# RapidAI/RapidDoc

Hardware: AMD Instinct MI355X
Metric: pages/sec (layout+OCR det/rec) (higher is better)
Workload: dtype f32

## Files before the change

### rapiddoc_amd/csrc/api.cpp

```cpp
#include "../../include/rapiddoc_mi355.h"

#include <mutex>
#include <string>

#include "engine.h"

namespace rd {
class FormulaDecoder;
FormulaDecoder* formula_decoder_create(int device, const void* blob, size_t nbytes);
void formula_decoder_destroy(FormulaDecoder* d);
int formula_decoder_decode(FormulaDecoder* d, const float* enc, int B, int S, int max_new, long long* ids, hipStream_t s);
int formula_decoder_max_new(FormulaDecoder* d);
}

struct rd_handle {
    rd::Engine* eng = nullptr;
    rd::FormulaDecoder* dec = nullptr;
    int device = 0;
    std::string kind;
    std::string err;
    std::string prof;
};

static thread_local std::string g_create_err;
// ... 209 lines not shown
    p.pages = pages; p.H = H; p.W = W; p.page_stride = (size_t)H * W * 3;
    p.descs = reinterpret_cast<const rd::LineCropDesc*>(descs); p.n = n;
    p.scratch = scratch; p.max_crop_pixels = (long)max_crop_pixels;
    if (rd::launch_line_warp(p, (hipStream_t)stream) != 0) return 1;
    return hipGetLastError() == hipSuccess ? 0 : 1;
}
int rd_line_resize_norm_batch(int device_id, const rd_line_crop_desc* descs, int n, const uint8_t* scratch, int out_h, int out_w_padded,
                              int swap_rb, float* out, void* stream) {
    if (!descs || !scratch || !out || n < 0 || out_h <= 0 || out_w_padded <= 0) return 1;
    if (hipSetDevice(device_id) != hipSuccess) return 1;
    rd::LineCropParams p{};
    p.descs = reinterpret_cast<const rd::LineCropDesc*>(descs); p.n = n;
    p.scratch = const_cast<uint8_t*>(scratch);
    p.dst = out; p.OH = out_h; p.OWp = out_w_padded; p.swap_rb = swap_rb;
    if (rd::launch_line_resize_norm(p, (hipStream_t)stream) != 0) return 1;
    return hipGetLastError() == hipSuccess ? 0 : 1;
}

int rd_ctc_collapse(int device_id, const int32_t* idx, const float* prob, int B, int T, const uint8_t* ctab, int max_len, int n_classes,
                    uint8_t* out, int row_bytes, void* stream) {
    if (!idx || !prob || !ctab || !out || B < 0 || T <= 0 || max_len <= 0 || n_classes <= 0) return 1;
    if (hipSetDevice(device_id) != hipSuccess) return 1;
    if (rd::launch_ctc_collapse(idx, prob, B, T, nullptr, ctab, max_len, n_classes, out, row_bytes, nullptr, nullptr, (hipStream_t)stream) != 0) return 1;
    return hipGetLastError() == hipSuccess ? 0 : 1;
}

int rd_ctc_collapse_lines(int device_id, const int32_t* idx, const float* prob, int n_lines, const int32_t* seg, int max_tokens,
                          const uint8_t* ctab, int max_len, int n_classes, uint8_t* out, int row_bytes, uint16_t* kept_cols, float* kept_conf,
                          void* stream) {
    if (!idx || !prob || !seg || !ctab || !out || n_lines < 0 || max_tokens <= 0 || max_len <= 0 || n_classes <= 0) return 1;
    if (hipSetDevice(device_id) != hipSuccess) return 1;
    if (rd::launch_ctc_collapse(idx, prob, n_lines, max_tokens, seg, ctab, max_len, n_classes, out, row_bytes, kept_cols, kept_conf,
                                (hipStream_t)stream) != 0)
        return 1;
    return hipGetLastError() == hipSuccess ? 0 : 1;
}

int rd_msdeform_attn(int device_id, const float* value, const int32_t* shapes, const int32_t* level_start, const float* loc, const float* attn,
                     float* out, int B, int S, int H, int D, int Q, int L, int P, void* stream) {
    if (!value || !shapes || !level_start || !loc || !attn || !out || B < 0 || S <= 0 || H <= 0 || D <= 0 || Q < 0 || L <= 0 || P <= 0 || H * D > 1024)
        return 1;
    if (hipSetDevice(device_id) != hipSuccess) return 1;
    rd::launch_msdeform_attn(value, shapes, level_start, loc, attn, out, B, S, H, D, Q, L, P, (hipStream_t)stream);
    return hipGetLastError() == hipSuccess ? 0 : 1;
}

int rd_topk_rows(int device_id, const float* scores, int rows, int n, int k, float* out_vals, int32_t* out_idx, void* stream) {
    if (!scores || !out_vals || !out_idx || rows < 0 || n <= 0 || k <= 0 || k > 1024 || k > n) return 1;
    if (hipSetDevice(device_id) != hipSuccess) return 1;
    rd::launch_topk_rows(scores, rows, n, k, out_vals, out_idx, (hipStream_t)stream);
    return hipGetLastError() == hipSuccess ? 0 : 1;
}

size_t rd_encoder_layer_workspace(int M, int Dm, int F) {
    if (M <= 0 || Dm <= 0 || F <= 0) return 0;
    return ((size_t)M * Dm * 3  + (size_t)M * 3 * Dm  + (size_t)M * F) * sizeof(float);
}

int rd_encoder_layer(int device_id, const float* x, const float* pos, int B, int T, int Dm, int heads, int F, int act, const float* in_w,
                     const float* in_b, const float* out_w, const float* out_b, const float* ln1_g, const float* ln1_b, const float* w1,
                     const float* b1, const float* w2, const float* b2, const float* ln2_g, const float* ln2_b, float eps, float* out, void* ws,
                     size_t ws_bytes, void* stream) {
    const int M = B * T;
    if (!x || !in_w || !out_w || !w1 || !w2 || !ln1_g || !ln1_b || !ln2_g || !ln2_b || !out || !ws || B <= 0 || T <= 0 || heads <= 0 ||
        Dm % heads != 0 || Dm % 4 != 0 || F % 4 != 0 || ws_bytes < rd_encoder_layer_workspace(M, Dm, F))
        return 1;
    const int hd = Dm / heads;
    if (hd != 16 && hd != 32) return 1;
    if (hipSetDevice(device_id) != hipSuccess) return 1;
    hipStream_t s = (hipStream_t)stream;
    float* xp = (float*)ws;
    float* att = xp + (size_t)M * Dm;
    float* y1 = att + (size_t)M * Dm;
    float* qkv = y1 + (size_t)M * Dm;
    float* ff = qkv + (size_t)M * 3 * Dm;
    auto gemm = [&](const float* a, int K, const float* w, const float* b, int N, float* y, int yld, int a_act, const float* res) {
        rd::ConvParams p{};
        p.x = a; p.xld = K; p.N = 1; p.H = 1; p.W = M; p.Cin = K;
        p.w = w; p.bias = b; p.y = y; p.yld = yld; p.OH = 1; p.OW = M; p.Cout = N;
        p.KH = p.KW = p.SH = p.SW = 1;
        p.res = res; p.rld = N;
        p.act = a_act; p.out_mode = rd::OUT_NHWC;
        p.M = M; p.K = K; p.Ng = N;
        rd::launch_conv_igemm(p, s);
    };
    try {
        const float* qk_in = x;
        if (pos) {
            rd::launch_add(x, Dm, pos, Dm, xp, Dm, M, Dm, s);
            qk_in = xp;
        }
        gemm(qk_in, Dm, in_w, in_b, 2 * Dm, qkv, 3 * Dm, rd::ACT_NONE, nullptr);
        gemm(x, Dm, in_w + (size_t)2 * Dm * Dm, in_b ? in_b + 2 * Dm : nullptr, Dm, qkv + 2 * Dm, 3 * Dm, rd::ACT_NONE, nullptr);
        rd::launch_attention(qkv, att, B, T, heads, hd, 1.0f / std::sqrt((float)hd), s);
        gemm(att, Dm, out_w, out_b, Dm, xp, Dm, rd::ACT_NONE, x);
        rd::launch_layernorm(xp, Dm, y1, Dm, ln1_g, ln1_b, M, Dm, eps, s);
        gemm(y1, Dm, w1, b1, F, ff, F, act, nullptr);
        gemm(ff, F, w2, b2, Dm, xp, Dm, rd::ACT_NONE, y1);
        rd::launch_layernorm(xp, Dm, out, Dm, ln2_g, ln2_b, M, Dm, eps, s);
    } catch (...) {
        return 1;
    }
    return hipGetLastError() == hipSuccess ? 0 : 1;
}

size_t rd_db_boxes_workspace(int B, int H, int W, int max_runs, int max_candidates) {
    (void)W;
    if (B <= 0 || H <= 0 || max_runs <= 0 || max_candidates <= 0) return 0;
    return rd::db_boxes_workspace_bytes(B, H, max_runs, max_candidates);
}
int rd_db_boxes_device(int device_id, const float* prob, int B, int H, int W, const int32_t* src_hw_dev, float thresh, float box_thresh,
                       float unclip_ratio, int use_dilation, int max_candidates, int max_runs, void* ws, size_t ws_bytes, rd_text_box* out,
                       int max_out, int32_t* n_out, void* stream) {
    if (!prob || !src_hw_dev || !ws || !out || !n_out || B < 0 || H <= 0 || W <= 0) return 1;
    if (hipSetDevice(device_id) != hipSuccess) return 1;
    if (rd::launch_db_boxes(prob, B, H, W, src_hw_dev, thresh, box_thresh, unclip_ratio, use_dilation, max_candidates, max_runs, ws, ws_bytes,
                            out, max_out, n_out, (hipStream_t)stream) != 0)
        return 1;
    return hipGetLastError() == hipSuccess ? 0 : 1;
}

float rd_debug_time_mixer(int C, int M, int variant, int iters, float* x, float* y, float* w1, float* b1, float* w2, float* b2) {
    rd::MixerParams p{};
    p.x = x; p.xld = C; p.y = y; p.yld = C; p.M = M; p.HW = M; p.C = C; p.gate = nullptr;
    p.w1 = w1; p.b1 = b1; p.w2 = w2; p.b2 = b2;
    hipEvent_t e0, e1;
    (void)hipEventCreate(&e0); (void)hipEventCreate(&e1);
    void* hbuf[4] = {nullptr, nullptr, nullptr, nullptr};
    int ws_abl = 0;
    if (variant >= 1000) { ws_abl = (variant - 1000) & ~0xff; variant = 200 + ((variant - 1000) & 0xff); }
    if (variant >= 600) variant -= 300;
    if (variant >= 300 && variant < 400) {
        std::vector<float> hw1((size_t)2 * C * C), hw2((size_t)2 * C * C);
        (void)hipMemcpy(hw1.data(), w1, hw1.size() * 4, hipMemcpyDeviceToHost);
        (void)hipMemcpy(hw2.data(), w2, hw2.size() * 4, hipMemcpyDeviceToHost);
        std::vector<uint16_t> img;
        float inv[2];
        rd::prepare_mixer_weights_res(hw1.data(), hw2.data(), C, img, inv);
        p.ws_inv1 = inv[0]; p.ws_inv2 = inv[1];
        (void)hipMalloc(&hbuf[0], img.size() * 2);
        (void)hipMemcpy(hbuf[0], img.data(), img.size() * 2, hipMemcpyHostToDevice);
        p.w1h = (const uint16_t*)hbuf[0];
    } else if (variant >= 200) {
        const bool pf = variant >= 400 && variant < 600;
        if (pf) variant -= 200;
        p.ws_pf = pf;
        p.dbg = (variant - 200) | ws_abl;
        std::vector<float> hw1((size_t)2 * C * C), hw2((size_t)2 * C * C);
        (void)hipMemcpy(hw1.data(), w1, hw1.size() * 4, hipMemcpyDeviceToHost);
        (void)hipMemcpy(hw2.data(), w2, hw2.size() * 4, hipMemcpyDeviceToHost);
        std::vector<uint16_t> img;
        float inv[2];
        rd::prepare_mixer_weights_ws(hw1.data(), hw2.data(), C, img, inv);
        p.ws_inv1 = inv[0]; p.ws_inv2 = inv[1];
        (void)hipMalloc(&hbuf[0], img.size() * 2);
        (void)hipMemcpy(hbuf[0], img.data(), img.size() * 2, hipMemcpyHostToDevice);
        p.w1h = (const uint16_t*)hbuf[0];
    } else if (variant >= 100) {
        p.dbg = variant - 100;
        std::vector<float> hw1((size_t)2 * C * C), hw2((size_t)2 * C * C);
        (void)hipMemcpy(hw1.data(), w1, hw1.size() * 4, hipMemcpyDeviceToHost);
        (void)hipMemcpy(hw2.data(), w2, hw2.size() * 4, hipMemcpyDeviceToHost);
        std::vector<uint16_t> v[4];
        rd::prepare_mixer_weights_h3(hw1.data(), hw2.data(), C, v[0], v[1], v[2], v[3]);
        for (int i = 0; i < 4; ++i) {
            (void)hipMalloc(&hbuf[i], v[i].size() * 2);
            (void)hipMemcpy(hbuf[i], v[i].data(), v[i].size() * 2, hipMemcpyHostToDevice);
        }
        p.w1h = (const uint16_t*)hbuf[0]; p.w1l = (const uint16_t*)hbuf[1];
        p.w2h = (const uint16_t*)hbuf[2]; p.w2l = (const uint16_t*)hbuf[3];
    }
    auto go = [&] {
        if (variant >= 300 && !p.ws_pf) rd::launch_mixer_fused_res(p, nullptr);
        else if (variant >= 200) rd::launch_mixer_fused_ws(p, nullptr);
        else if (variant >= 100) rd::launch_mixer_fused_h3(p, nullptr);
        else rd::launch_mixer_debug(p, variant, nullptr);
    };
    go();
    (void)hipEventRecord(e0, nullptr);
    for (int i = 0; i < iters; ++i) go();
    (void)hipEventRecord(e1, nullptr);
    (void)hipEventSynchronize(e1);
    float ms = 0.f;
    (void)hipEventElapsedTime(&ms, e0, e1);
    (void)hipEventDestroy(e0); (void)hipEventDestroy(e1);
    for (void* b : hbuf) if (b) (void)hipFree(b);
    return ms / iters;
}
static bool debug_h1_image(const float* w_dev, int N, int K, void** img_dev, float* inv) {
    if (!rd::gemm_h1_shape_ok(K, N)) return false;
    std::vector<float> hw((size_t)N * K);
    if (hipMemcpy(hw.data(), w_dev, hw.size() * 4, hipMemcpyDeviceToHost) != hipSuccess) return false;
    std::vector<uint16_t> img;
    *inv = rd::prepare_gemm_h1_weights(hw.data(), N, K, img);
    if (hipMalloc(img_dev, img.size() * 2) != hipSuccess) return false;
    (void)hipMemcpy(*img_dev, img.data(), img.size() * 2, hipMemcpyHostToDevice);
    return true;
}
float rd_debug_time_gemm(int M, int K, int N, int act, int iters, float* x, float* w, float* b, float* y, void* wh, void* wl) {
    rd::ConvParams p{};
    p.wh = (const uint16_t*)wh; p.wl = (const uint16_t*)wl;
    p.x = x; p.xld = K; p.N = 1; p.H = 1; p.W = M; p.Cin = K; p.w = w; p.bias = b; p.y = y; p.yld = N;
    p.OH = 1; p.OW = M; p.Cout = N; p.KH = p.KW = p.SH = p.SW = 1; p.act = act; p.out_mode = rd::OUT_NHWC;
    p.M = M; p.K = K; p.Ng = N;
    void* img = nullptr;
    float inv = 0.f;
    if (wh && debug_h1_image(w, N, K, &img, &inv)) { p.w1 = (const uint16_t*)img; p.w1_inv = inv; }
    hipEvent_t e0, e1;
    (void)hipEventCreate(&e0); (void)hipEventCreate(&e1);
    auto go = [&] { if (wh) rd::launch_conv_igemm_h3(p, nullptr); else rd::launch_conv_igemm(p, nullptr); };
    go();
    (void)hipEventRecord(e0, nullptr);
    for (int i = 0; i < iters; ++i) go();
    (void)hipEventRecord(e1, nullptr);
    (void)hipEventSynchronize(e1);
    float ms = 0.f;
    (void)hipEventElapsedTime(&ms, e0, e1);
    (void)hipEventDestroy(e0); (void)hipEventDestroy(e1);
    if (img) (void)hipFree(img);
    return ms / iters;
}
float rd_debug_gemm_h1(int M, int K, int N, int act, int iters, float* x, int xld, float* w, float* b, float* res, int rld, float* y, int yld,
                       int* range_out) {
    rd::ConvParams p{};
    p.x = x; p.xld = xld; p.N = 1; p.H = 1; p.W = M; p.Cin = K; p.w = w; p.bias = b; p.y = y; p.yld = yld;
    p.OH = 1; p.OW = M; p.Cout = N; p.KH = p.KW = p.SH = p.SW = 1; p.act = act; p.out_mode = rd::OUT_NHWC;
    p.res = res; p.rld = rld;
    p.M = M; p.K = K; p.Ng = N;
    void* img = nullptr;
    float inv = 0.f;
    if (!debug_h1_image(w, N, K, &img, &inv)) return -1.f;
    p.w1 = (const uint16_t*)img; p.w1_inv = inv;
    unsigned* flag = nullptr;
    (void)hipHostMalloc((void**)&flag, sizeof(unsigned), hipHostMallocMapped);
    *flag = 0;
    p.range_flag = flag;
    float ms = -1.f;
    if (rd::gemm_h1_applies(p)) {
        hipEvent_t e0, e1;
        (void)hipEventCreate(&e0); (void)hipEventCreate(&e1);
        rd::launch_gemm_h1(p, nullptr);
        (void)hipEventRecord(e0, nullptr);
        for (int i = 0; i < iters; ++i) rd::launch_gemm_h1(p, nullptr);
        (void)hipEventRecord(e1, nullptr);
        (void)hipEventSynchronize(e1);
        (void)hipEventElapsedTime(&ms, e0, e1);
        (void)hipEventDestroy(e0); (void)hipEventDestroy(e1);
        ms = iters > 0 ? ms / iters : 0.f;
    }
    (void)hipDeviceSynchronize();
    if (range_out) *range_out = (int)*flag;
    (void)hipHostFree(flag);
    (void)hipFree(img);
    return ms;
}

float rd_debug_conv(int N, int H, int W, int Cin, int Cout, int KH, int KW, int S, int PT, int PL, int PB, int PR, int act, int iters,
                    float* x, float* w, void* wh, void* wl, float* bias, float* res, float* y, int* used_direct) {
    rd::ConvParams p{};
    p.x = x; p.xld = Cin; p.N = N; p.H = H; p.W = W; p.Cin = Cin; p.w = w; p.bias = bias; p.y = y; p.yld = Cout;
    p.wh = (const uint16_t*)wh; p.wl = (const uint16_t*)wl;
    p.OH = (H + PT + PB - KH) / S + 1; p.OW = (W + PL + PR - KW) / S + 1; p.Cout = Cout;
    p.KH = KH; p.KW = KW; p.SH = p.SW = S; p.PT = PT; p.PL = PL; p.act = act; p.out_mode = rd::OUT_NHWC;
    p.res = res; p.rld = Cout;
    p.M = N * p.OH * p.OW; p.K = KH * KW * Cin; p.Ng = Cout;
    void* img3 = nullptr;
    if (wh && !(used_direct && *used_direct) && rd::conv3x3_h1_shape_ok(KH, KW, Cin, Cout)) {
        std::vector<float> hw((size_t)Cout * p.K);
        if (hipMemcpy(hw.data(), w, hw.size() * 4, hipMemcpyDeviceToHost) == hipSuccess) {
            std::vector<uint16_t> img;
            const float inv = rd::prepare_conv3x3_h1_weights(hw.data(), Cout, Cin, img);
            if (hipMalloc(&img3, img.size() * 2) == hipSuccess) {
                (void)hipMemcpy(img3, img.data(), img.size() * 2, hipMemcpyHostToDevice);
                p.w3 = (const uint16_t*)img3;
                p.w3_inv = inv;
            }
        }
    }
    const bool c3 = wh && rd::conv3x3_h1_applies(p);
    const bool force = used_direct && *used_direct == 1 && wh && rd::conv_direct_h3_supported(p);
    const bool force_stream = used_direct && *used_direct == 2 && wh && rd::conv_stream_h3_supported(p);
    if (used_direct) *used_direct = c3 ? 3 : force_stream ? 2 : (force || (wh && !rd::conv_stream_h3_applies(p) && rd::conv_direct_h3_applies(p))) ? 1
                                    : (wh && rd::conv_stream_h3_applies(p)) ? 2 : 0;
    hipEvent_t e0, e1;
    (void)hipEventCreate(&e0); (void)hipEventCreate(&e1);
    auto go = [&] {
        if (force_stream) rd::launch_conv_stream_h3(p, nullptr);
        else if (force) rd::launch_conv_direct_h3(p, nullptr);
        else if (wh) rd::launch_conv_igemm_h3(p, nullptr);
        else rd::launch_conv_igemm(p, nullptr);
    };
    go();
    (void)hipEventRecord(e0, nullptr);
    for (int i = 0; i < iters; ++i) go();
    (void)hipEventRecord(e1, nullptr);
    (void)hipEventSynchronize(e1);
    float ms = 0.f;
    (void)hipEventElapsedTime(&ms, e0, e1);
    (void)hipEventDestroy(e0); (void)hipEventDestroy(e1);
    if (img3) (void)hipFree(img3);
    return iters > 0 ? ms / iters : 0.f;
}

float rd_debug_stem34(int N, int H, int W, int Cin, int xld, int N1, int N2, int yld, int act3, int act4, int iters, float* x, float* w3, float* b3,
                      float* w4, float* b4, float* y, unsigned* range_flag) {
    if (!rd::stem34_shape_ok(Cin, N1, N2)) return -1.f;
    std::vector<float> h3((size_t)N1 * 9 * Cin), h4((size_t)N2 * N1), hb3((size_t)((N1 + 31) / 32) * 32, 0.f);
    if (hipMemcpy(h3.data(), w3, h3.size() * 4, hipMemcpyDeviceToHost) != hipSuccess) return -1.f;
    if (hipMemcpy(h4.data(), w4, h4.size() * 4, hipMemcpyDeviceToHost) != hipSuccess) return -1.f;
    if (hipMemcpy(hb3.data(), b3, (size_t)N1 * 4, hipMemcpyDeviceToHost) != hipSuccess) return -1.f;
    std::vector<uint16_t> i3, i4;
    float inv[2];
    rd::prepare_stem34_weights(h3.data(), h4.data(), Cin, N1, N2, i3, i4, inv);
    void *d3 = nullptr, *d4 = nullptr, *db3 = nullptr;
    if (hipMalloc(&d3, i3.size() * 2) != hipSuccess || hipMalloc(&d4, i4.size() * 2) != hipSuccess || hipMalloc(&db3, hb3.size() * 4) != hipSuccess) return -1.f;
    (void)hipMemcpy(d3, i3.data(), i3.size() * 2, hipMemcpyHostToDevice);
    (void)hipMemcpy(d4, i4.data(), i4.size() * 2, hipMemcpyHostToDevice);
    (void)hipMemcpy(db3, hb3.data(), hb3.size() * 4, hipMemcpyHostToDevice);
    rd::Stem34Params p{};
    p.x = x; p.xld = xld; p.N = N; p.H = H; p.W = W; p.Cin = Cin; p.y = y; p.yld = yld;
    p.OH = (H - 1) / 2 + 1; p.OW = (W - 1) / 2 + 1; p.N1 = N1; p.N2 = N2;
    p.w3 = (const uint16_t*)d3; p.w3_inv = inv[0]; p.b3 = (const float*)db3;
    p.w4 = (const uint16_t*)d4; p.w4_inv = inv[1]; p.b4 = b4;
    p.act3 = act3; p.act4 = act4; p.range_flag = range_flag;
    hipEvent_t e0, e1;
    (void)hipEventCreate(&e0); (void)hipEventCreate(&e1);
    rd::launch_stem34(p, nullptr);
    (void)hipEventRecord(e0, nullptr);
    for (int i = 0; i < iters; ++i) rd::launch_stem34(p, nullptr);
    (void)hipEventRecord(e1, nullptr);
    (void)hipEventSynchronize(e1);
    float ms = 0.f;
    (void)hipEventElapsedTime(&ms, e0, e1);
    (void)hipEventDestroy(e0); (void)hipEventDestroy(e1);
    (void)hipFree(d3); (void)hipFree(d4); (void)hipFree(db3);
    return iters > 0 ? ms / iters : 0.f;
}

float rd_debug_dwconv(int N, int H, int W, int C, int K, int SH, int act, int iters, float* x, float* w, float* bias, float* res, float* y,
                      const int32_t* line_w, float* gap, int* gap_chunks) {
    rd::DwParams p{};
    p.x = x; p.xld = C; p.N = N; p.H = H; p.W = W; p.C = C; p.w = w; p.bias = bias; p.y = y; p.yld = C;
    p.KH = p.KW = K; p.SH = SH; p.SW = 1; p.PT = p.PL = K / 2;
    p.OH = (H + 2 * p.PT - K) / SH + 1; p.OW = W; p.act = act; p.res = res; p.rld = C;
    const int chunks = rd::dwconv_gap_chunks(p);
    if (gap_chunks) *gap_chunks = chunks;
    p.gap_partial = chunks > 0 ? gap : nullptr; p.gap_chunks = chunks;
    p.line_w = line_w; p.line_w_stride = 1;
    if (gap_chunks && rd::dwconv_kxk_lds_applies(p)) *gap_chunks = -1;
    hipEvent_t e0, e1;
    (void)hipEventCreate(&e0); (void)hipEventCreate(&e1);
    rd::launch_dwconv(p, nullptr);
    (void)hipEventRecord(e0, nullptr);
    for (int i = 0; i < iters; ++i) rd::launch_dwconv(p, nullptr);
    (void)hipEventRecord(e1, nullptr);
    (void)hipEventSynchronize(e1);
    float ms = 0.f;
    (void)hipEventElapsedTime(&ms, e0, e1);
    (void)hipEventDestroy(e0); (void)hipEventDestroy(e1);
    return iters > 0 ? ms / iters : 0.f;
}

float rd_debug_time_ctc(int M, int K, int Ccls, int iters, float* x, float* wp, void* wh, void* wl, float* part, int32_t* idx, float* prob,
                        int nsplit_override, int* nsplit_out) {
    rd::CtcParams p{};
    p.x = x; p.xld = K; p.w = wp; p.M = M; p.K = K; p.C = Ccls; p.part = part;
    p.nsplit = nsplit_override > 0 ? nsplit_override : rd::ctc_head_nsplit(M, Ccls, wh != nullptr);
    p.idx = idx; p.prob = prob;
    p.wh = (const uint16_t*)wh; p.wl = (const uint16_t*)wl;
    if (nsplit_out) *nsplit_out = p.nsplit;
    hipEvent_t e0, e1;
    (void)hipEventCreate(&e0); (void)hipEventCreate(&e1);
    rd::launch_ctc_head(p, nullptr);
    (void)hipEventRecord(e0, nullptr);
    for (int i = 0; i < iters; ++i) rd::launch_ctc_head(p, nullptr);
    (void)hipEventRecord(e1, nullptr);
    (void)hipEventSynchronize(e1);
    float ms = 0.f;
    (void)hipEventElapsedTime(&ms, e0, e1);
    (void)hipEventDestroy(e0); (void)hipEventDestroy(e1);
    return ms / iters;
}

int rd_set_precision(rd_handle* h, const char* mode) {
    return guarded(h, [&] {
        RD_CHECK(h->eng, "precision modes apply to the network engines");
        const std::string m = mode ? mode : "";
        RD_CHECK(m == "auto" || m == "fp32" || m == "h3", "precision must be auto, fp32 or h3");
        h->eng->set_precision(m == "h3" ? rd::Engine::PREC_H3 : m == "fp32" ? rd::Engine::PREC_FP32 : rd::Engine::PREC_AUTO);
    });
}
int rd_range_status(rd_handle* h, void* stream) {
    int out = 0;
    const int rc = guarded(h, [&] { if (h->eng) out = h->eng->take_range_flag((hipStream_t)stream); });
    return rc != 0 ? -1 : out;
}

int rd_plan_stats(rd_handle* h, uint64_t* plans_built, uint64_t* graph_captures, uint64_t* graph_replays) {
    if (!h || !h->eng) return 1;
    if (plans_built) *plans_built = h->eng->plans_built();
    if (graph_captures) *graph_captures = h->eng->graph_captures();
    if (graph_replays) *graph_replays = h->eng->graph_replays();
    return 0;
}

int rd_set_profiling(rd_handle* h, int on) {
    return guarded(h, [&] { if (h->eng) h->eng->set_profiling(on != 0); });
}
const char* rd_profile_json(rd_handle* h) {
    if (!h || !h->eng) return "[]";
    h->prof = h->eng->profile_json();
    return h->prof.c_str();
}

}
```

### rapiddoc_amd/csrc/engine.cpp

```cpp
#include "engine.h"

#include <algorithm>
#include <cmath>
#include <cstdio>
#include <cstdlib>
#include <cstring>
#include <sstream>

namespace rd {

namespace {
struct JsonCur {
    const char* p;
    const char* end;
    void ws() {
        while (p < end && (*p == ' ' || *p == '\n' || *p == '\t' || *p == '\r')) ++p;
    }
    bool eat(char c) {
        ws();
        if (p < end && *p == c) { ++p; return true; }
        return false;
    }
    void expect(char c) {
        if (!eat(c)) throw Error(std::string("safetensors header: expected '") + c + "'");
// ... 383 lines not shown
            pb_->add_u16(key + "#w3", img);
            pb_->add(key + "#w3s", std::vector<float>{inv});
        }
        if (kh == 1 && kw == 1 && gemm_h1_shape_ok(K, cout)) {
            std::vector<uint16_t> img;
            const float inv = prepare_gemm_h1_weights(wf.data(), cout, K, img);
            pb_->add_u16(key + "#w1", img);
            pb_->add(key + "#w1s", std::vector<float>{inv});
        }
    }
}

bool Builder::mixer_takes_dw(const std::string& prefix, int C) const {
    if (!planning() || !(h3_ || mixer_h3_) || !mixer_res_fuses_dw(C)) return false;
    const std::string hkey = prefix + ".mixer#h3";
    static const bool ws_off = std::getenv("RD_MIXER_WS") && std::string(std::getenv("RD_MIXER_WS")) == "0";
    const bool split = pb_->has(hkey + ".w1h");
    const bool ws = split && !ws_off && pb_->has(hkey + ".ws");
    return split && !ws && pb_->has(hkey + ".res");
}

TView Builder::mixer_fused(const std::string& prefix, const TView& x, const TView* gate, const std::string* dw_key) {
    const std::string w1 = prefix + ".channel_conv1.convolution.weight", bn1 = prefix + ".channel_conv1.normalization";
    const std::string w2 = prefix + ".channel_conv2.convolution.weight", bn2 = prefix + ".channel_conv2.normalization";
    const int C = x.c;
    RD_CHECK(mixer_fused_supported(C), "mixer_fused: unsupported width");
    RD_CHECK(weight_dim(w1, 0) == 2 * C && weight_dim(w1, 1) == C && weight_dim(w2, 0) == C && weight_dim(w2, 1) == 2 * C,
             "mixer_fused: weight shapes: " + prefix);
    TView y = alloc(x.n, x.h, x.w, C);
    const std::string hkey = prefix + ".mixer#h3";
    if (!planning()) {
        fold_conv(w1, "", bn1);
        fold_conv(w2, "", bn2);
        const float* f1 = pb_->host_ptr(w1 + "|" + bn1 + "#w");
        const float* f2 = pb_->host_ptr(w2 + "|" + bn2 + "#w");
        const bool fits = fits_fp16_range(std::vector<float>(f1, f1 + (size_t)2 * C * C)) && fits_fp16_range(std::vector<float>(f2, f2 + (size_t)2 * C * C));
        if (!pb_->has(hkey + ".w1h") && fits) {
            std::vector<uint16_t> v[4];
            prepare_mixer_weights_h3(f1, f2, C, v[0], v[1], v[2], v[3]);
            pb_->add_u16(hkey + ".w1h", v[0]); pb_->add_u16(hkey + ".w1l", v[1]);
            pb_->add_u16(hkey + ".w2h", v[2]); pb_->add_u16(hkey + ".w2l", v[3]);
        }
        if (!pb_->has(hkey + ".res") && fits && mixer_res_supported(C)) {
            std::vector<uint16_t> img;
            float inv[2];
            prepare_mixer_weights_res(f1, f2, C, img, inv);
            pb_->add_u16(hkey + ".res", img);
            pb_->add(hkey + ".resinv", std::vector<float>{inv[0], inv[1]});
        }
        if (!pb_->has(hkey + ".ws") && fits && mixer_ws_preferred(C)) {
            std::vector<uint16_t> img;
            float inv[2];
            prepare_mixer_weights_ws(f1, f2, C, img, inv);
            pb_->add_u16(hkey + ".ws", img);
            pb_->add(hkey + ".wsinv", std::vector<float>{inv[0], inv[1]});
        }
        return y;
    }
    const bool split = (h3_ || mixer_h3_) && pb_->has(hkey + ".w1h");
    static const bool ws_off = std::getenv("RD_MIXER_WS") && std::string(std::getenv("RD_MIXER_WS")) == "0";
    const bool ws = split && !ws_off && pb_->has(hkey + ".ws");
    const bool res_k = split && !ws && mixer_res_supported(C) && pb_->has(hkey + ".res");
    MixerParams p{};
    if (res_k) {
        p.w1h = reinterpret_cast<const uint16_t*>(pb_->ptr(hkey + ".res"));
        p.ws_inv1 = pb_->host_ptr(hkey + ".resinv")[0];
        p.ws_inv2 = pb_->host_ptr(hkey + ".resinv")[1];
        p.range_flag = range_flag_;
    } else if (ws) {
        p.w1h = reinterpret_cast<const uint16_t*>(pb_->ptr(hkey + ".ws"));
        p.ws_inv1 = pb_->host_ptr(hkey + ".wsinv")[0];
        p.ws_inv2 = pb_->host_ptr(hkey + ".wsinv")[1];
        p.ws_pf = mixer_ws_prefetch() && C == 192;
        p.range_flag = range_flag_;
    } else if (split) {
        p.w1h = reinterpret_cast<const uint16_t*>(pb_->ptr(hkey + ".w1h")); p.w1l = reinterpret_cast<const uint16_t*>(pb_->ptr(hkey + ".w1l"));
        p.w2h = reinterpret_cast<const uint16_t*>(pb_->ptr(hkey + ".w2h")); p.w2l = reinterpret_cast<const uint16_t*>(pb_->ptr(hkey + ".w2l"));
        p.range_flag = range_flag_;
    }
    p.xld = plan_->ld(x);
    p.yld = plan_->ld(y);
    p.M = (int)x.pixels(); p.HW = x.h * x.w; p.C = C;
    const bool with_dw = dw_key != nullptr;
    if (with_dw) {
        RD_CHECK(res_k && !gate, "mixer_fused: the depthwise conv only rides in the resident-weights kernel, without a gate: " + prefix);
        RD_CHECK((size_t)x.pixels() * plan_->ld(x) < ((size_t)1 << 29), "mixer_fused + depthwise: the input tensor exceeds the 32-bit tap offsets");
        p.dw_w = pb_->ptr(*dw_key + "#w");
        p.dw_b = pb_->ptr(*dw_key + "#b");
        p.dwH = x.h; p.dwW = x.w;
    }
    p.w1 = pb_->ptr(w1 + "|" + bn1 + "#w"); p.b1 = pb_->ptr(w1 + "|" + bn1 + "#b");
    p.w2 = pb_->ptr(w2 + "|" + bn2 + "#w"); p.b2 = pb_->ptr(w2 + "|" + bn2 + "#b");
    OpRecord r;
    r.name = prefix + ".mixer";
    r.kind = res_k ? (with_dw ? "mixer_fused_res_dw" : "mixer_fused_res") : ws ? "mixer_fused_ws" : split ? "mixer_fused_h3" : "mixer_fused";
    r.cfg = "C" + std::to_string(C);
    r.shape = "M" + std::to_string(p.M) + "_C" + std::to_string(C);
    r.flops = 8.0 * p.M * (double)C * C + (with_dw ? 18.0 * p.M * C : 0.0);
    r.bytes = 8.0 * p.M * C;
    const TView xv = x, yv = y;
    const bool has_gate = gate != nullptr;
    const TView gv = gate ? *gate : TView{};
    const bool has_lt = with_dw && has_lt_;
    const TView ltv = lt_;
    r.run = [p, xv, yv, gv, has_gate, split, ws, res_k, has_lt, ltv](const Plan& pl, const RunCtx& c) {
        MixerParams q = p;
        q.x = pl.vptr(xv, c);
        q.y = pl.vptr(yv, c);
        q.gate = has_gate ? pl.vptr(gv, c) : nullptr;
        if (has_lt) {
            q.dw_line_w = reinterpret_cast<const int32_t*>(pl.vptr(ltv, c)) + 2;
            q.dw_line_w_stride = kLineTabStride;
        }
        if (res_k) launch_mixer_fused_res(q, c.stream);
        else if (ws) launch_mixer_fused_ws(q, c.stream);
        else if (split) launch_mixer_fused_h3(q, c.stream);
        else launch_mixer_fused(q, c.stream);
    };
    emit(std::move(r));
    return y;
}

TView Builder::linear(const std::string& prefix, const TView& x, int act, const TView* out, const TView* res) {
    return conv(prefix + ".weight", has_weight(prefix + ".bias") ? prefix + ".bias" : "", "", x, ConvGeom{}, act, out, res);
}

bool Builder::deconv_pair_to_prob(const std::string& w1n, const std::string& b1n, const std::string& bn1, const std::string& w2n,
                                  const std::string& b2n, const TView& x, const TView& out) {
    static const bool off = [] { const char* e = getenv("RD_DET_HEAD_FUSED"); return e && e[0] == '0'; }();
    const HostTensor& w1 = ws_->get(w1n);
    const HostTensor& w2 = ws_->get(w2n);
    if (off || w1.shape.size() != 4 || w2.shape.size() != 4 || w1.shape[2] != 2 || w1.shape[3] != 2 || w2.shape[2] != 2 || w2.shape[3] != 2)
        return false;
    const int cin = (int)w1.shape[0], cmid = (int)w1.shape[1], cout = (int)w2.shape[1];
    if (!det_head_tail_supported(cin, cmid, cout) || (int)w2.shape[0] != cmid || cin != x.c) return false;
    RD_CHECK(out.h == 4 * x.h && out.w == 4 * x.w && out.c == 1 && out.n == x.n, "det head tail: output view mismatch");
    const std::string key = w1n + "|" + bn1 + "|" + w2n + "|pair";
    if (!planning()) {
        if (!pb_->has(key + "#w1")) {
            std::vector<float> shift;
            std::vector<float> scale = bn_scale_shift(bn1, cmid, shift);
            std::vector<float> wa((size_t)4 * cmid * cin), ba(cmid, 0.f), wb((size_t)4 * cmid), bb(1, 0.f);
            const float* s1 = w1.f32();
            for (int ci = 0; ci < cin; ++ci)
                for (int co = 0; co < cmid; ++co)
                    for (int tap = 0; tap < 4; ++tap)
                        wa[((size_t)tap * cmid + co) * cin + ci] = s1[((size_t)ci * cmid + co) * 4 + tap] * scale[co];
            if (!b1n.empty()) {
                const float* bs = ws_->get(b1n).f32();
                for (int co = 0; co < cmid; ++co) ba[co] = bs[co] * scale[co];
            }
            for (int co = 0; co < cmid; ++co) ba[co] += shift[co];
            const float* s2 = w2.f32();
            for (int co = 0; co < cmid; ++co)
                for (int tap = 0; tap < 4; ++tap) wb[(size_t)tap * cmid + co] = s2[(size_t)co * 4 + tap];
            if (!b2n.empty()) bb[0] = ws_->get(b2n).f32()[0];
            pb_->add(key + "#w1", wa);
            pb_->add(key + "#b1", ba);
            pb_->add(key + "#w2", wb);
            pb_->add(key + "#b2", bb);
        }
        return true;
    }
    const float* pw1 = pb_->ptr(key + "#w1");
    const float* pb1 = pb_->ptr(key + "#b1");
    const float* pw2 = pb_->ptr(key + "#w2");
    const float* pb2 = pb_->ptr(key + "#b2");
    OpRecord r;
    r.name = w1n + "+" + w2n;
    r.kind = "det_head_tail";
    r.cfg = "fused";
    const double m = (double)x.n * x.h * x.w;
    r.flops = 2.0 * m * (4.0 * cmid * cin + 16.0 * cmid);
    r.bytes = 4.0 * (m * cin + m * 16);
    const TView xv = x, yv = out;
    r.run = [xv, yv, pw1, pb1, pw2, pb2](const Plan& pl, const RunCtx& c) {
        launch_det_head_tail(pl.vptr(xv, c), pl.ld(xv), xv.n, xv.h, xv.w, pw1, pb1, pw2, pb2, pl.vptr(yv, c), c.stream);
    };
    emit(std::move(r));
    return true;
}

TView Builder::deconv2x2(const std::string& wname, const std::string& bname, const std::string& bn, const TView& x,
                         int act, const TView* out) {
    const HostTensor& w = ws_->get(wname);
    RD_CHECK(w.shape.size() == 4 && w.shape[2] == 2 && w.shape[3] == 2, "deconv2x2 weight shape: " + wname);
    const int cin = (int)w.shape[0], cout = (int)w.shape[1];
    RD_CHECK(cin == x.c && cin % 4 == 0, "deconv Cin mismatch: " + wname);
    TView y = out ? *out : alloc(x.n, 2 * x.h, 2 * x.w, cout);
    RD_CHECK(y.h == 2 * x.h && y.w == 2 * x.w && y.c == cout, "deconv output view mismatch");
    const std::string key = wname + "|" + bn + "|T";
    if (!planning()) {
        if (!pb_->has(key + "#w")) {
            std::vector<float> shift;
            std::vector<float> scale = bn_scale_shift(bn, cout, shift);
            std::vector<float> wf((size_t)4 * cout * cin);
            const float* src = w.f32();
            for (int ci = 0; ci < cin; ++ci)
                for (int co = 0; co < cout; ++co)
                    for (int dy = 0; dy < 2; ++dy)
                        for (int dx = 0; dx < 2; ++dx)
                            wf[((size_t)(dy * 2 + dx) * cout + co) * cin + ci] =
                                src[(((size_t)ci * cout + co) * 2 + dy) * 2 + dx] * scale[co];
            std::vector<float> bias(cout, 0.f);
            if (!bname.empty()) {
                const float* bs = ws_->get(bname).f32();
                for (int co = 0; co < cout; ++co) bias[co] = bs[co] * scale[co];
            }
            for (int co = 0; co < cout; ++co) bias[co] += shift[co];
            pb_->add(key + "#w", wf);
            pb_->add(key + "#b", bias);
            if (h3_ && fits_fp16_range(wf)) {
                std::vector<uint16_t> hi, lo;
                split_weights_h3(wf.data(), 4 * cout, cin, hi, lo);
                pb_->add_u16(key + "#wh", hi);
                pb_->add_u16(key + "#wl", lo);
            }
        }
        return y;
    }
    ConvParams p{};
    p.xld = plan_->ld(x);
    p.N = x.n; p.H = x.h; p.W = x.w; p.Cin = cin;
    p.w = pb_->ptr(key + "#w");
    p.bias = pb_->ptr(key + "#b");
    if (h3_ && pb_->has(key + "#wh")) {
        p.wh = reinterpret_cast<const uint16_t*>(pb_->ptr(key + "#wh"));
        p.wl = reinterpret_cast<const uint16_t*>(pb_->ptr(key + "#wl"));
        p.range_flag = range_flag_;
    }
    p.yld = plan_->ld(y);
    p.OH = x.h; p.OW = x.w; p.Cout = cout;
    p.KH = p.KW = p.SH = p.SW = 1;
    p.act = act;
    p.out_mode = OUT_DECONV2X2;
    p.M = x.n * x.h * x.w; p.K = cin; p.Ng = 4 * cout;
    OpRecord r;
    r.name = wname;
    r.kind = "deconv2x2";
    r.cfg = conv_igemm_config_name(p);
    r.flops = 2.0 * p.M * (double)cin * 4 * cout;
    r.bytes = 4.0 * ((double)p.M * cin + (double)p.M * 4 * cout);
    const TView xv = x, yv = y;
    const bool h3 = h3_ && p.wh != nullptr;
    r.run = [p, xv, yv, h3](const Plan& pl, const RunCtx& c) {
        ConvParams q = p;
        q.x = pl.vptr(xv, c);
        q.y = pl.vptr(yv, c);
        if (h3) launch_conv_igemm_h3(q, c.stream);
        else launch_conv_igemm(q, c.stream);
    };
    emit(std::move(r));
    return y;
}

TView Builder::stem3x3s2(const std::string& wname, const std::string& bn, const TView& xin, int act) {
    const HostTensor& w = ws_->get(wname);
    RD_CHECK(w.shape.size() == 4 && w.shape[1] == 3 && w.shape[2] == 3 && w.shape[3] == 3, "stem weight shape");
    const int cout = (int)w.shape[0];
    RD_CHECK(cout % 8 == 0, "stem Cout % 8");
    const int oh = out_dim(xin.h, 3, 2, 1, 1), ow = out_dim(xin.w, 3, 2, 1, 1);
    TView y = alloc(xin.n, oh, ow, cout);
    const std::string key = wname + "|" + bn + "|stem";
    if (!planning()) {
        if (!pb_->has(key + "#w")) {
            std::vector<float> shift;
            std::vector<float> scale = bn_scale_shift(bn, cout, shift);
            std::vector<float> wf((size_t)27 * cout);
            const float* src = w.f32();
            for (int co = 0; co < cout; ++co)
                for (int ci = 0; ci < 3; ++ci)
                    for (int a = 0; a < 3; ++a)
                        for (int b = 0; b < 3; ++b)
                            wf[(size_t)((a * 3 + b) * 3 + ci) * cout + co] = src[(((size_t)co * 3 + ci) * 3 + a) * 3 + b] * scale[co];
            pb_->add(key + "#w", wf);
            pb_->add(key + "#b", shift);
        }
        return y;
    }
    StemParams p{};
    p.N = xin.n; p.H = xin.h; p.W = xin.w; p.in_ch = xin.c;
    p.w = pb_->ptr(key + "#w");
    p.bias = pb_->ptr(key + "#b");
    p.yld = plan_->ld(y);
    p.OH = oh; p.OW = ow; p.Cout = cout;
    p.act = act;
    OpRecord r;
    r.name = wname;
    r.kind = "stem3x3s2";
    r.flops = 2.0 * xin.n * oh * ow * 27.0 * cout;
    r.bytes = 4.0 * ((double)xin.n * xin.c * xin.h * xin.w + (double)xin.n * oh * ow * cout);
    const TView xv = xin, yv = y;
    r.run = [p, xv, yv](const Plan& pl, const RunCtx& c) {
        StemParams q = p;
        q.x = pl.vptr(xv, c);
        q.y = pl.vptr(yv, c);
        launch_stem_conv3x3s2(q, c.stream);
    };
    emit(std::move(r));
    return y;
}

TView Builder::stem_front(const std::string& w1, const std::string& bn1, const std::string& w2a, const std::string& bn2a,
                          const std::string& w2b, const std::string& bn2b, const TView& xin) {
    const int c1 = weight_dim(w1, 0);
    ConvGeom g2;
    g2.kh = g2.kw = 2;
    g2.pb = g2.pr = 1;
    const std::string fkey = w1 + "|" + bn1 + "|stemfront";
    const bool off = std::getenv("RD_STEM_FUSED") && std::getenv("RD_STEM_FUSED")[0] == '0';
    const bool fused = planning() && !off && (h3_ || mixer_h3_) && pb_->has(fkey + "#img");
    if (!fused) {
        TView e = stem3x3s2(w1, bn1, xin, ACT_RELU);
        mask_cols(e, 1);
        TView a = conv(w2a, "", bn2a, e, g2, ACT_RELU);
        mask_cols(a, 1);
        TView cat = alloc(e.n, e.h, e.w, 2 * c1);
        TView cat_pool = slice(cat, 0, c1), cat_b = slice(cat, c1, c1);
        maxpool2x2s1(e, cat_pool);
        conv(w2b, "", bn2b, a, g2, ACT_RELU, &cat_b);
        mask_cols(cat_b, 1);
        release(e);
        release(a);
        if (!planning() && stem_fused_supported(c1) && !pb_->has(fkey + "#img")) {
            const std::string k1 = w1 + "|" + bn1 + "|stem", k2a = w2a + "|" + bn2a, k2b = w2b + "|" + bn2b;
            const float* f1 = pb_->host_ptr(k1 + "#w");
            const float* f2a = pb_->host_ptr(k2a + "#w");
            const float* f2b = pb_->host_ptr(k2b + "#w");
            const int na = c1 / 2;
            const bool fits = fits_fp16_range(std::vector<float>(f1, f1 + (size_t)27 * c1)) &&
                              fits_fp16_range(std::vector<float>(f2a, f2a + (size_t)na * 4 * c1)) &&
                              fits_fp16_range(std::vector<float>(f2b, f2b + (size_t)c1 * 4 * na));
            if (fits && weight_dim(w2a, 0) == na && weight_dim(w2a, 1) == c1 && weight_dim(w2b, 0) == c1 && weight_dim(w2b, 1) == na) {
                std::vector<uint16_t> img;
                prepare_stem_fused_weights(c1, f1, f2a, f2b, img);
                pb_->add_u16(fkey + "#img", img);
                std::vector<float> bias;
                const float* b1 = pb_->host_ptr(k1 + "#b");
                bias.insert(bias.end(), b1, b1 + c1);
                const float* b2a = pb_->host_ptr(k2a + "#b");
                bias.insert(bias.end(), b2a, b2a + na);
                const float* b2b = pb_->host_ptr(k2b + "#b");
                bias.insert(bias.end(), b2b, b2b + c1);
                pb_->add(fkey + "#bias", bias);
            }
        }
        return cat;
    }
    const int oh = out_dim(xin.h, 3, 2, 1, 1), ow = out_dim(xin.w, 3, 2, 1, 1);
    TView cat = alloc(xin.n, oh, ow, 2 * c1);
    const uint16_t* img = reinterpret_cast<const uint16_t*>(pb_->ptr(fkey + "#img"));
    const float* bias = pb_->ptr(fkey + "#bias");
    OpRecord r;
    r.name = w1 + ":front";
    r.kind = "stem_fused";
    r.cfg = "C" + std::to_string(c1);
    r.shape = "N" + std::to_string(xin.n) + "_" + std::to_string(oh) + "x" + std::to_string(ow);
    const int na = c1 / 2;
    r.flops = 2.0 * xin.n * oh * ow * (27.0 * c1 + 4.0 * c1 * na + 4.0 * na * c1);
    r.bytes = 4.0 * ((double)xin.n * xin.c * xin.h * xin.w + (double)xin.n * oh * ow * 2 * c1);
    const TView xv = xin, yv = cat;
    unsigned* flag = range_flag_;
    const bool has_lt = has_lt_;
    const TView ltv = lt_;
    r.run = [xv, yv, img, bias, c1, flag, has_lt, ltv](const Plan& pl, const RunCtx& c) {
        launch_stem_fused(c1, pl.vptr(xv, c), xv.n, xv.h, xv.w, xv.c, img, bias, pl.vptr(yv, c), pl.ld(yv), flag, c.stream,
                          has_lt ? reinterpret_cast<const int32_t*>(pl.vptr(ltv, c)) : nullptr);
    };
    emit(std::move(r));
    return cat;
}

TView Builder::stem_tail(const std::string& w3, const std::string& bn3, const std::string& w4, const std::string& bn4, const TView& x, int act3,
                         int act4, const TView* out) {
    const int n1 = weight_dim(w3, 0), cin = weight_dim(w3, 1), n2 = weight_dim(w4, 0);
    ConvGeom g3;
    g3.kh = g3.kw = 3;
    g3.sh = g3.sw = 2;
    g3.pt = g3.pl = g3.pb = g3.pr = 1;
    ConvGeom g1;
    const std::string fkey = w3 + "|" + bn3 + "|" + w4 + "|" + bn4 + "|stemtail";
    const int oh = out_dim(x.h, 3, 2, 1, 1), ow = out_dim(x.w, 3, 2, 1, 1);
    const bool fused = planning() && stem34_enabled() && (h3_ || mixer_h3_) && pb_->has(fkey + "#w3") && plan_->ld(x) % 4 == 0 &&
                       (size_t)x.h * x.w * plan_->ld(x) < ((size_t)1 << 30) && (!out || (plan_->ld(*out) % 4 == 0 && out->coff % 4 == 0)) &&
                       (size_t)oh * ow * (out ? plan_->ld(*out) : n2) < ((size_t)1 << 29);
    if (!fused) {
        TView s3 = conv(w3, "", bn3, x, g3, act3);
        TView s4 = conv(w4, "", bn4, s3, g1, act4, out);
        release(s3);
        if (!planning() && stem34_enabled() && !pb_->has(fkey + "#w3") && stem34_shape_ok(cin, n1, n2) && weight_dim(w3, 2) == 3 && weight_dim(w3, 3) == 3 &&
            weight_dim(w4, 1) == n1) {
            const std::string k3 = w3 + "|" + bn3, k4 = w4 + "|" + bn4;
            const float* f3 = pb_->host_ptr(k3 + "#w");
            const float* f4 = pb_->host_ptr(k4 + "#w");
            if (fits_fp16_range(std::vector<float>(f3, f3 + (size_t)n1 * 9 * cin)) && fits_fp16_range(std::vector<float>(f4, f4 + (size_t)n2 * n1))) {
                std::vector<uint16_t> img3, img4;
                float inv[2];
                prepare_stem34_weights(f3, f4, cin, n1, n2, img3, img4, inv);
                pb_->add_u16(fkey + "#w3", img3);
                pb_->add_u16(fkey + "#w4", img4);
                std::vector<float> b3((size_t)((n1 + 31) / 32) * 32, 0.f), b4((size_t)n2, 0.f);
                if (pb_->has(k3 + "#b")) std::copy(pb_->host_ptr(k3 + "#b"), pb_->host_ptr(k3 + "#b") + n1, b3.begin());
                if (pb_->has(k4 + "#b")) std::copy(pb_->host_ptr(k4 + "#b"), pb_->host_ptr(k4 + "#b") + n2, b4.begin());
                pb_->add(fkey + "#b3", b3);
                pb_->add(fkey + "#b4", b4);
                pb_->add(fkey + "#inv", std::vector<float>{inv[0], inv[1]});
            }
        }
        return s4;
    }
    TView y = out ? *out : alloc(x.n, oh, ow, n2);
    RD_CHECK(y.n == x.n && y.h == oh && y.w == ow && y.c == n2, "stem_tail output view mismatch: " + w4);
    Stem34Params p{};
    p.xld = plan_->ld(x);
    p.N = x.n; p.H = x.h; p.W = x.w; p.Cin = cin;
    p.yld = plan_->ld(y);
    p.OH = oh; p.OW = ow; p.N1 = n1; p.N2 = n2;
    p.w3 = reinterpret_cast<const uint16_t*>(pb_->ptr(fkey + "#w3"));
    p.w4 = reinterpret_cast<const uint16_t*>(pb_->ptr(fkey + "#w4"));
    p.b3 = pb_->ptr(fkey + "#b3");
    p.b4 = pb_->ptr(fkey + "#b4");
    p.w3_inv = pb_->host_ptr(fkey + "#inv")[0];
    p.w4_inv = pb_->host_ptr(fkey + "#inv")[1];
    p.act3 = act3; p.act4 = act4;
    p.range_flag = range_flag_;
    OpRecord r;
    r.name = w3 + ":tail";
    r.kind = "stem_tail";
    r.cfg = "C" + std::to_string(cin) + "_" + std::to_string(n1) + "_" + std::to_string(n2);
    r.shape = "M" + std::to_string(x.n * oh * ow) + "_K" + std::to_string(9 * cin) + "_N" + std::to_string(n1) + "_N" + std::to_string(n2);
    r.flops = 2.0 * x.n * oh * ow * (9.0 * cin * n1 + (double)n1 * n2);
    r.bytes = 4.0 * ((double)x.pixels() * cin + (double)x.n * oh * ow * n2 + 9.0 * cin * n1 + (double)n1 * n2);
    const TView xv = x, yv = y;
    r.run = [p, xv, yv](const Plan& pl, const RunCtx& c) mutable {
        Stem34Params q = p;
        q.x = pl.vptr(xv, c);
        q.y = pl.vptr(yv, c);
        launch_stem34(q, c.stream);
    };
    emit(std::move(r));
    return y;
}

void Builder::mask_cols(const TView& v, int col) {
    if (!has_lt_ || !planning()) return;
    OpRecord r;
    r.name = "mask_cols";
    r.kind = "mask";
    r.bytes = 4.0 * v.pixels() * v.c;
    const TView yv = v, ltv = lt_;
    r.run = [yv, ltv, col](const Plan& pl, const RunCtx& c) {
        launch_mask_cols(pl.vptr(yv, c), pl.ld(yv), yv.n, yv.h, yv.w, yv.c, reinterpret_cast<const int32_t*>(pl.vptr(ltv, c)) + col,
                         kLineTabStride, c.stream);
    };
    emit(std::move(r));
}

TView Builder::dwconv(const std::string& wname, const std::string& bname, const std::string& bn, const TView& x,
                      const ConvGeom& g, int act, const TView* out, const TView* res, GapOut* gap, const TView* tokinfo) {
    const HostTensor& w = ws_->get(wname);
    RD_CHECK(w.shape.size() == 4 && w.shape[1] == 1, "depthwise weight shape: " + wname);
    const int c = (int)w.shape[0], kh = (int)w.shape[2], kw = (int)w.shape[3];
    RD_CHECK(c == x.c && c % 4 == 0, "depthwise channel mismatch: " + wname);
    RD_CHECK(kh == g.kh && kw == g.kw, "depthwise kernel mismatch: " + wname);
    const int oh = out_dim(x.h, kh, g.sh, g.pt, g.pb), ow = out_dim(x.w, kw, g.sw, g.pl, g.pr);
    TView y = out ? *out : alloc(x.n, oh, ow, c);
    RD_CHECK(y.h == oh && y.w == ow && y.c == c, "depthwise output view mismatch: " + wname);
    const std::string key = wname + "|" + bn + "|dw";
    if (gap) {
        DwParams gp{};
        gp.N = x.n; gp.H = x.h; gp.W = x.w; gp.C = c; gp.OH = oh; gp.OW = ow;
        gp.KH = kh; gp.KW = kw; gp.SH = g.sh; gp.SW = g.sw; gp.PT = g.pt; gp.PL = g.pl;
        gap->chunks = dwconv_gap_chunks(gp);
        if (gap->chunks > 0) gap->partial = alloc_raw((size_t)x.n * gap->chunks * c);
    }
    if (!planning()) {
        if (!pb_->has(key + "#w")) {
            std::vector<float> shift;
            std::vector<float> scale = bn_scale_shift(bn, c, shift);
            std::vector<float> wf((size_t)kh * kw * c);
            const float* src = w.f32();
            for (int ch = 0; ch < c; ++ch)
                for (int t = 0; t < kh * kw; ++t) wf[(size_t)t * c + ch] = src[(size_t)ch * kh * kw + t] * scale[ch];
            std::vector<float> bias(c, 0.f);
            if (!bname.empty()) {
                const float* bs = ws_->get(bname).f32();
                for (int ch = 0; ch < c; ++ch) bias[ch] = bs[ch] * scale[ch];
            }
            for (int ch = 0; ch < c; ++ch) bias[ch] += shift[ch];
            pb_->add(key + "#w", wf);
            pb_->add(key + "#b", bias);
        }
        return y;
    }
    DwParams p{};
    p.xld = plan_->ld(x);
    p.N = x.n; p.H = x.h; p.W = x.w; p.C = c;
    p.w = pb_->ptr(key + "#w");
    p.bias = pb_->ptr(key + "#b");
    p.yld = plan_->ld(y);
    p.OH = oh; p.OW = ow; p.KH = kh; p.KW = kw; p.SH = g.sh; p.SW = g.sw; p.PT = g.pt; p.PL = g.pl;
    p.act = act;
    p.rld = res ? plan_->ld(*res) : 0;
    OpRecord r;
    r.name = wname;
    r.kind = "dwconv" + std::to_string(kh) + "x" + std::to_string(kw);
    r.flops = 2.0 * x.n * oh * ow * (double)c * kh * kw;
    r.bytes = 4.0 * ((double)x.pixels() * c + (double)x.n * oh * ow * c * (res ? 2 : 1));
    const TView xv = x, yv = y;
    const bool has_res = res != nullptr;
    const TView rv = res ? *res : TView{};
    const bool has_gap = gap && gap->chunks > 0;
    const TView gpv = has_gap ? gap->partial : TView{};
    const bool ragged = tokinfo != nullptr;
    RD_CHECK(!ragged || (kh == 1 && g.sw == 1 && x.n == 1 && x.h == 1 && x.w < (1 << 30)), "ragged depthwise conv: 1 x k over one token row");
    const TView tiv = ragged ? *tokinfo : TView{};
    const bool has_lt = has_lt_ && !ragged;
    RD_CHECK(!has_lt || (g.sw == 1 && ow == x.w), "line table: depthwise convs keep the width (stride (s, 1), 'same' padding)");
    const TView ltv = lt_;
    r.run = [p, xv, yv, rv, has_res, has_gap, gpv, ragged, tiv, has_lt, ltv](const Plan& pl, const RunCtx& cx) {
        DwParams q = p;
        q.x = pl.vptr(xv, cx);
        q.y = pl.vptr(yv, cx);
        q.res = has_res ? pl.vptr(rv, cx) : nullptr;
        q.gap_partial = has_gap ? pl.vptr(gpv, cx) : nullptr;
        q.tokinfo = ragged ? reinterpret_cast<const int32_t*>(pl.vptr(tiv, cx)) : nullptr;
        if (has_lt) {
            q.line_w = reinterpret_cast<const int32_t*>(pl.vptr(ltv, cx)) + 2;
            q.line_w_stride = kLineTabStride;
        }
        launch_dwconv(q, cx.stream);
    };
    emit(std::move(r));
    return y;
}

void Builder::maxpool2x2s1(const TView& x, const TView& out) {
    RD_CHECK(out.h == x.h && out.w == x.w && out.c == x.c && x.c % 4 == 0, "maxpool view mismatch");
    if (!planning()) return;
    OpRecord r;
    r.name = "maxpool2x2s1";
    r.kind = "pool";
    r.bytes = 8.0 * x.pixels() * x.c;
    const TView xv = x, yv = out;
    r.run = [xv, yv](const Plan& pl, const RunCtx& c) {
        launch_maxpool2x2s1(pl.vptr(xv, c), pl.ld(xv), pl.vptr(yv, c), pl.ld(yv), xv.n, xv.h, xv.w, xv.c, c.stream);
    };
    emit(std::move(r));
}

TView Builder::avgpool3x2(const TView& x, const TView* out) {
    RD_CHECK(x.h >= 3 && x.w >= 2, "avg_pool2d([3,2]): feature map too small");
    const int oh = (x.h - 3) / 3 + 1, ow = (x.w - 2) / 2 + 1;
    TView y = out ? *out : alloc(x.n, oh, ow, x.c);
    RD_CHECK(y.n == x.n && y.h == oh && y.w == ow && y.c == x.c, "avgpool3x2: output view mismatch");
    if (!planning()) return y;
    OpRecord r;
    r.name = "avgpool3x2";
    r.kind = "pool";
    r.bytes = 4.0 * (x.pixels() * x.c + y.pixels() * y.c);
    const TView xv = x, yv = y;
    const bool has_lt = has_lt_;
    RD_CHECK(!has_lt || oh == 1, "line table: the pooled map is one row of tokens per line");
    const TView ltv = lt_;
    r.run = [xv, yv, has_lt, ltv](const Plan& pl, const RunCtx& c) {
        launch_avgpool3x2(pl.vptr(xv, c), pl.ld(xv), pl.vptr(yv, c), pl.ld(yv), xv.n, xv.h, xv.w, xv.c, c.stream,
                          has_lt ? reinterpret_cast<const int32_t*>(pl.vptr(ltv, c)) : nullptr);
    };
    emit(std::move(r));
    return y;
}

TView Builder::se_gate(const std::string& w1n, const std::string& b1n, const std::string& w2n, const std::string& b2n,
                       const TView& x, int gate_act, const GapOut* pre) {
    const HostTensor& w1 = ws_->get(w1n);
    const int cr = (int)w1.shape[0], c = (int)w1.shape[1];
    RD_CHECK(c == x.c && c % 4 == 0, "SE channel mismatch: " + w1n);
    RD_CHECK(c <= 512, "SE width above 512 channels (se_fc_kernel reads a row of W1 with two 16-byte loads per lane): " + w1n);
    const int hw = x.h * x.w;
    const bool fused_gap = pre && pre->chunks > 0;
    RD_CHECK(!has_lt_ || fused_gap, "line table: the SE pooling sums must come from the depthwise kernel (it leaves out the columns beyond a line)");
    const int chunks = fused_gap ? pre->chunks : std::max(1, std::min(64, hw / 256));
    TView partial = fused_gap ? pre->partial : alloc_raw((size_t)x.n * chunks * c);
    TView gate = alloc(x.n, 1, 1, c);
    if (!planning()) {
        if (!pb_->has(w1n)) {
            const HostTensor& w2 = ws_->get(w2n);
            pb_->add(w1n, std::vector<float>(w1.f32(), w1.f32() + w1.numel()));
            pb_->add(b1n, std::vector<float>(ws_->get(b1n).f32(), ws_->get(b1n).f32() + cr));
            pb_->add(w2n, std::vector<float>(w2.f32(), w2.f32() + w2.numel()));
            pb_->add(b2n, std::vector<float>(ws_->get(b2n).f32(), ws_->get(b2n).f32() + c));
        }
        release(partial);
        return gate;
    }
    if (!fused_gap) {
        OpRecord r;
        r.name = w1n + ":gap";
        r.kind = "gap";
        r.bytes = 4.0 * x.pixels() * c;
        const TView xv = x, pv = partial;
        r.run = [xv, pv, hw, c, chunks](const Plan& pl, const RunCtx& cx) {
            launch_gap_partial(pl.vptr(xv, cx), pl.ld(xv), xv.n, hw, c, pl.vptr(pv, cx), chunks, cx.stream);
        };
        emit(std::move(r));
    }
    {
        SeFcParams p{};
        p.chunks = chunks; p.N = x.n; p.C = c; p.Cr = cr; p.inv_hw = 1.f / (float)hw;
        p.w1 = pb_->ptr(w1n); p.b1 = pb_->ptr(b1n); p.w2 = pb_->ptr(w2n); p.b2 = pb_->ptr(b2n);
        p.gate = gate_act;
        OpRecord r;
        r.name = w1n + ":fc";
        r.kind = "se_fc";
        r.flops = 4.0 * x.n * c * cr;
        const TView pv = partial, gv = gate;
        const bool has_lt = has_lt_;
        const TView ltv = lt_;
        p.H = x.h;
        r.run = [p, pv, gv, has_lt, ltv](const Plan& pl, const RunCtx& cx) {
            SeFcParams q = p;
            q.partial = pl.vptr(pv, cx);
            q.scale = pl.vptr(gv, cx);
            if (has_lt) {
                q.line_w = reinterpret_cast<const int32_t*>(pl.vptr(ltv, cx)) + 2;
                q.line_w_stride = kLineTabStride;
            }
            launch_se_fc(q, cx.stream);
        };
        emit(std::move(r));
    }
    release(partial);
    return gate;
}

void Builder::scale(const TView& x, const TView& gate, float alpha, const TView& out) {
    RD_CHECK(out.h == x.h && out.w == x.w && out.c == x.c && gate.c == x.c, "scale view mismatch");
    if (!planning()) return;
    OpRecord r;
    r.name = "se_scale";
    r.kind = "scale";
    r.bytes = 8.0 * x.pixels() * x.c;
    const TView xv = x, gv = gate, yv = out;
    r.run = [xv, gv, yv, alpha](const Plan& pl, const RunCtx& c) {
        launch_scale_channels(pl.vptr(xv, c), pl.ld(xv), pl.vptr(yv, c), pl.ld(yv), pl.vptr(gv, c), alpha, xv.n,
                              xv.h * xv.w, xv.c, c.stream);
    };
    emit(std::move(r));
}

void Builder::upsample(const TView& x, const TView& out, int f, bool accumulate) {
    RD_CHECK(out.h == x.h * f && out.w == x.w * f && out.c == x.c && out.n == x.n, "upsample view mismatch");
    if (!planning()) return;
    OpRecord r;
    r.name = accumulate ? "upsample_add" : "upsample_copy";
    r.kind = "upsample";
    r.bytes = 4.0 * (x.pixels() * x.c + out.pixels() * out.c * (accumulate ? 2 : 1));
    const TView xv = x, yv = out;
    r.run = [xv, yv, f, accumulate](const Plan& pl, const RunCtx& c) {
        launch_upsample(pl.vptr(xv, c), pl.ld(xv), pl.vptr(yv, c), pl.ld(yv), yv.n, yv.h, yv.w, yv.c, f,
                        accumulate ? 1 : 0, c.stream);
    };
    emit(std::move(r));
}

TView Builder::layernorm(const std::string& prefix, const TView& x, float eps) {
    RD_CHECK(x.c <= 512, "layernorm: C <= 512");
    TView y = alloc(x.n, x.h, x.w, x.c);
    if (!planning()) {
        if (!pb_->has(prefix + ".weight")) {
            const HostTensor& g = ws_->get(prefix + ".weight");
            const HostTensor& b = ws_->get(prefix + ".bias");
            RD_CHECK((int)g.numel() == x.c, "layernorm width: " + prefix);
            pb_->add(prefix + ".weight", std::vector<float>(g.f32(), g.f32() + g.numel()));
            pb_->add(prefix + ".bias", std::vector<float>(b.f32(), b.f32() + b.numel()));
        }
        return y;
    }
    const float* g = pb_->ptr(prefix + ".weight");
    const float* b = pb_->ptr(prefix + ".bias");
    OpRecord r;
    r.name = prefix;
    r.kind = "layernorm";
    r.bytes = 8.0 * x.pixels() * x.c;
    const TView xv = x, yv = y;
    r.run = [xv, yv, g, b, eps](const Plan& pl, const RunCtx& c) {
        launch_layernorm(pl.vptr(xv, c), pl.ld(xv), pl.vptr(yv, c), pl.ld(yv), g, b, (int)xv.pixels(), xv.c, eps, c.stream);
    };
    emit(std::move(r));
    return y;
}

TView Builder::attention(const TView& qkv, int B, int T, int heads, int hd, const TView* seg) {
    RD_CHECK(qkv.c == 3 * heads * hd && qkv.coff == 0 && plan_->ld(qkv) == qkv.c, "attention: packed qkv expected");
    RD_CHECK(hd == 15 || hd == 16 || hd == 32, "attention: head_dim 15/16/32");
    TView o = alloc(qkv.n, qkv.h, qkv.w, heads * hd);
    if (!planning()) return o;
    const float sc = 1.0f / std::sqrt((float)hd);
    OpRecord r;
    r.name = "self_attn";
    r.kind = "attention";
    r.flops = 4.0 * B * heads * (double)T * T * hd;
    const TView qv = qkv, ov = o;
    const bool ragged = seg != nullptr;
    const TView sv = ragged ? *seg : TView{};
    r.run = [qv, ov, B, T, heads, hd, sc, ragged, sv](const Plan& pl, const RunCtx& c) {
        launch_attention(pl.vptr(qv, c), pl.vptr(ov, c), B, T, heads, hd, sc, c.stream,
                         ragged ? reinterpret_cast<const int32_t*>(pl.vptr(sv, c)) : nullptr);
    };
    emit(std::move(r));
    return o;
}

TView Builder::add(const TView& a, const TView& b) {
    RD_CHECK(a.pixels() == b.pixels() && a.c == b.c, "add: shape mismatch");
    TView y = alloc(a.n, a.h, a.w, a.c);
    if (!planning()) return y;
    OpRecord r;
    r.name = "add";
    r.kind = "add";
    r.bytes = 12.0 * a.pixels() * a.c;
    const TView av = a, bv = b, yv = y;
    r.run = [av, bv, yv](const Plan& pl, const RunCtx& c) {
        launch_add(pl.vptr(av, c), pl.ld(av), pl.vptr(bv, c), pl.ld(bv), pl.vptr(yv, c), pl.ld(yv), (int)av.pixels(), av.c, c.stream);
    };
    emit(std::move(r));
    return y;
}

void Builder::to_nchw(const TView& x, const TView& out_ext) {
// ... 386 lines not shown
```

### rapiddoc_amd/csrc/engine.h

```cpp
#pragma once
#include <hip/hip_runtime.h>

#include <cstdint>
#include <functional>
#include <map>
#include <memory>
#include <stdexcept>
#include <string>
#include <unordered_map>
#include <vector>

#include "rd_kernels.h"

namespace rd {

struct Error : std::runtime_error {
    using std::runtime_error::runtime_error;
};
#define RD_CHECK(cond, msg)                                                          \
    do {                                                                             \
        if (!(cond)) throw ::rd::Error(std::string(msg) + " [" #cond "]");           \
    } while (0)
#define RD_HIP(expr)                                                                                      \
    do {                                                                                                  \
        hipError_t _e = (expr);                                                                           \
        if (_e != hipSuccess) throw ::rd::Error(std::string(#expr ": ") + hipGetErrorString(_e));          \
    } while (0)

struct HostTensor {
    std::vector<int64_t> shape;
    std::string dtype;
    const uint8_t* data = nullptr;
    size_t nbytes = 0;
    size_t numel() const {
        size_t n = 1;
        for (auto d : shape) n *= (size_t)d;
        return n;
    }
    const float* f32() const { return reinterpret_cast<const float*>(data); }
};

class WeightStore {
   public:
    void load_safetensors(const void* blob, size_t nbytes);
    bool has(const std::string& name) const { return map_.count(name) != 0; }
    const HostTensor& get(const std::string& name) const;
    size_t size() const { return map_.size(); }
    void clear() { map_.clear(); blob_.clear(); blob_.shrink_to_fit(); }

   private:
    std::vector<uint8_t> blob_;
    std::unordered_map<std::string, HostTensor> map_;
};

class ParamBlock {
   public:
    ~ParamBlock();
    size_t add(const std::string& key, const std::vector<float>& v);
    size_t add_u16(const std::string& key, const std::vector<uint16_t>& v);
    bool has(const std::string& key) const { return off_.count(key) != 0; }
    void upload();
    const float* ptr(const std::string& key) const;
    const float* host_ptr(const std::string& key) const;
    size_t bytes() const { return host_.size() * sizeof(float); }

   private:
    std::vector<float> host_;
    std::unordered_map<std::string, size_t> off_;
    float* dev_ = nullptr;
};

struct Buf {
    int n = 0, h = 0, w = 0, c = 0;
    size_t off = 0, bytes = 0;
    int external = -1;
    bool live = false;
};
struct TView {
    int buf = -1, coff = 0;
    int n = 0, h = 0, w = 0, c = 0;
    long pixels() const { return (long)n * h * w; }
};

struct RunCtx {
    uint8_t* arena = nullptr;
    std::vector<void*> ext;
    hipStream_t stream = nullptr;
};

struct OpRecord {
    std::string name, kind, cfg, shape;
    double flops = 0, bytes = 0;
    std::function<void(const struct Plan&, const RunCtx&)> run;
};

struct GraphSlot {
    std::vector<void*> ext;
    uint8_t* arena = nullptr;
    hipStream_t stream = nullptr;
    hipGraphExec_t exec = nullptr;
    uint64_t last_use = 0;
};

struct Plan {
    ~Plan();
    std::vector<Buf> bufs;
    std::vector<OpRecord> ops;
    size_t arena_bytes = 0;
    mutable uint64_t last_use = 0;
    mutable std::vector<GraphSlot> graphs;
    mutable bool graph_broken = false;
    mutable unsigned graph_evictions = 0;
    std::vector<TView> outputs;
    float* vptr(const TView& v, const RunCtx& c) const {
        const Buf& b = bufs[v.buf];
        uint8_t* base = b.external >= 0 ? (uint8_t*)c.ext[b.external] : c.arena + b.off;
        return reinterpret_cast<float*>(base) + v.coff;
    }
    int ld(const TView& v) const { return bufs[v.buf].c; }
};

struct ProfileEntry {
    std::string name, kind, cfg, shape;
    double flops, bytes;
    float ms;
};

enum class Mode { PREPARE, PLAN };

class Builder {
   public:
    Builder(Mode m, const WeightStore* ws, ParamBlock* pb, Plan* plan, bool h3 = false, bool mixer_h3 = false,
            unsigned* range_flag = nullptr)
        : mode_(m), h3_(h3), mixer_h3_(mixer_h3), range_flag_(range_flag), ws_(ws), pb_(pb), plan_(plan) {}
    bool h3() const { return h3_; }
    Mode mode() const { return mode_; }
    bool planning() const { return mode_ == Mode::PLAN; }

    TView alloc(int n, int h, int w, int c);
    TView external(int slot, int n, int h, int w, int c);
    TView slice(const TView& v, int coff, int c) const;
    TView reshape(const TView& v, int n, int h, int w) const;
    void release(const TView& v);
    TView alloc_raw(size_t nfloats);

    void set_line_table(const TView& t) { lt_ = t; has_lt_ = true; }
    void mask_cols(const TView& v, int col);

    struct ConvGeom {
        int kh = 1, kw = 1, sh = 1, sw = 1, pt = 0, pl = 0, pb = 0, pr = 0;
    };
    TView conv(const std::string& wname, const std::string& bname, const std::string& bn, const TView& x,
               const ConvGeom& g, int act, const TView* out = nullptr, const TView* res = nullptr,
               const TView* ascale = nullptr);
    TView mixer_fused(const std::string& prefix, const TView& x, const TView* gate, const std::string* dw_key = nullptr);
    bool mixer_takes_dw(const std::string& prefix, int C) const;
    static std::string dw_key(const std::string& wname, const std::string& bn) { return wname + "|" + bn + "|dw"; }
    void fold_conv(const std::string& wname, const std::string& bname, const std::string& bn);
    TView linear(const std::string& prefix, const TView& x, int act, const TView* out = nullptr,
                 const TView* res = nullptr);
    bool deconv_pair_to_prob(const std::string& w1n, const std::string& b1n, const std::string& bn1, const std::string& w2n,
                             const std::string& b2n, const TView& x, const TView& out);
    TView deconv2x2(const std::string& wname, const std::string& bname, const std::string& bn, const TView& x, int act,
                    const TView* out = nullptr);
    TView stem3x3s2(const std::string& wname, const std::string& bn, const TView& x_nchw, int act);
    TView stem_front(const std::string& w1, const std::string& bn1, const std::string& w2a, const std::string& bn2a,
                     const std::string& w2b, const std::string& bn2b, const TView& x_nchw);
    TView stem_tail(const std::string& w3, const std::string& bn3, const std::string& w4, const std::string& bn4, const TView& x, int act3,
                    int act4, const TView* out = nullptr);
    struct GapOut { TView partial; int chunks = 0; };
    TView dwconv(const std::string& wname, const std::string& bname, const std::string& bn, const TView& x,
                 const ConvGeom& g, int act, const TView* out = nullptr, const TView* res = nullptr, GapOut* gap = nullptr,
                 const TView* tokinfo = nullptr);
    void maxpool2x2s1(const TView& x, const TView& out);
    TView avgpool3x2(const TView& x, const TView* out = nullptr);
    TView se_gate(const std::string& w1, const std::string& b1, const std::string& w2, const std::string& b2,
                  const TView& x, int gate_act, const GapOut* pre = nullptr);
    void scale(const TView& x, const TView& gate, float alpha, const TView& out);
    void upsample(const TView& x, const TView& out, int f, bool accumulate);
    TView layernorm(const std::string& prefix, const TView& x, float eps);
    TView attention(const TView& qkv, int B, int T, int heads, int hd, const TView* seg = nullptr);
    TView add(const TView& a, const TView& b);
    void to_nchw(const TView& x, const TView& out_ext);
    void copy(const TView& x, const TView& out);
    void ctc_stats(const TView& logits, const TView& idx_ext, const TView& prob_ext);
    void softmax_rows(const TView& logits, const TView& out_ext, const TView* idx_ext = nullptr, const TView* prob_ext = nullptr);
    void ctc_head(const std::string& prefix, const TView& x, const TView& idx_ext, const TView& prob_ext);

    const HostTensor& weight(const std::string& name) const { return ws_->get(name); }
    bool has_weight(const std::string& name) const { return ws_ && ws_->has(name); }
    int weight_dim(const std::string& name, int d) const;

   private:
    void emit(OpRecord&& r) { plan_->ops.push_back(std::move(r)); }
    std::vector<float> bn_scale_shift(const std::string& bn, int c, std::vector<float>& shift) const;
    Mode mode_;
    bool h3_ = false;
    bool mixer_h3_ = false;
    unsigned* range_flag_ = nullptr;
    const WeightStore* ws_;
    ParamBlock* pb_;
    Plan* plan_;
    struct Block { size_t off, size; bool free; };
    std::vector<Block> blocks_;
    TView lt_;
    bool has_lt_ = false;
};

class Engine {
   public:
    explicit Engine(int device, const std::string& kind);
    ~Engine();
    const std::string& kind() const { return kind_; }
    void load_weights(const void* blob, size_t nbytes);
    bool loaded() const { return loaded_; }

    const Plan& plan_for(int B, int H, int W, int flags = 0);
    size_t workspace_bytes(int B, int H, int W, int flags = 0) { return plan_for(B, H, W, flags).arena_bytes; }
    void run(int B, int H, int W, int flags, const std::vector<void*>& ext, void* ws, size_t ws_bytes, hipStream_t s);

    uint64_t plans_built() const { return plans_built_; }
    uint64_t graph_captures() const { return graph_captures_; }
    uint64_t graph_replays() const { return graph_replays_; }
    void set_profiling(bool on) { profiling_ = on; }
    const std::vector<ProfileEntry>& last_profile() const { return profile_; }
    std::string profile_json() const;
    int n_classes() const { return n_classes_; }
    int rec_token_dim() const { return rec_token_dim_; }
    bool h3() const { return precision_ == PREC_H3; }
    int device() const { return device_; }
    enum Precision : int { PREC_AUTO = 0, PREC_FP32 = 1, PREC_H3 = 2 };
    void set_precision(int p);
    int precision() const { return precision_; }
    int take_range_flag(hipStream_t s);

    std::string last_error;

   private:
    void build(Builder& b, int B, int H, int W, int flags);
    int device_;
    std::string kind_;
    bool loaded_ = false;
    bool profiling_ = false;
    int precision_ = PREC_AUTO;
    bool h3_prepared_ = false;
    unsigned* range_flag_ = nullptr;
    unsigned* range_flag_host_ = nullptr;
    int n_classes_ = 0;
    int rec_token_dim_ = 0;
    ParamBlock params_;
    WeightStore store_;
    std::map<std::tuple<int, int, int, int>, std::unique_ptr<Plan>> plans_;
    uint64_t plan_clock_ = 0;
    uint64_t plans_built_ = 0, graph_captures_ = 0, graph_replays_ = 0;
    static constexpr size_t kMaxPlans = 512;
    static constexpr size_t kMaxGraphSlots = 8;
    static constexpr unsigned kMaxGraphEvictions = 32;
    struct RetiredGraph { hipGraphExec_t exec; hipEvent_t done; };
    std::vector<RetiredGraph> retired_graphs_;
    void retire_graph(hipGraphExec_t exec, hipStream_t s);
    void sweep_retired_graphs(bool wait);
    bool graphs_ = true;
    uint8_t* arena_ = nullptr;
    size_t arena_bytes_ = 0;
    std::vector<ProfileEntry> profile_;
    std::vector<hipEvent_t> events_;
};

void build_ppocrv6_det(Builder& b, int B, int H, int W);
enum RecFlags : int { REC_UNFUSED_CTC = 1, REC_WANT_SOFTMAX = 2, REC_WANT_LOGITS = 4, REC_STAGE_BACKBONE = 8, REC_STAGE_TAIL = 16, REC_LINE_WIDTHS = 32 };
void build_ppocrv6_rec(Builder& b, int B, int H, int W, int flags);
void build_pphgnetv2_b4(Builder& b, int B, int H, int W);
void build_pphgnetv2_b6_formula(Builder& b, int B, int H, int W, int flags);

}
```

### rapiddoc_amd/csrc/kernels_stem34.hip

```cpp
#include <algorithm>
#include <cmath>
#include <cstdlib>
#include <type_traits>
#include <vector>

#include "rd_device.h"

namespace rd {

static constexpr int S34_WAVES = 4;
static constexpr int S34_SLAB_STEPS = 9;

typedef _Float16 s34_f16x2 __attribute__((ext_vector_type(2)));
__device__ __forceinline__ void s34_split4(const f32x4 v, float neg1, f16x4& hi, f16x4& lo) {
#pragma unroll
    for (int e = 0; e < 4; e += 2) {
        const s34_f16x2 h = __builtin_convertvector(f32x2{v[e], v[e + 1]}, s34_f16x2);
        hi[e] = h[0];
        hi[e + 1] = h[1];
        lo[e] = (_Float16)__builtin_fmaf((float)h[0], neg1, v[e]);
        lo[e + 1] = (_Float16)__builtin_fmaf((float)h[1], neg1, v[e + 1]);
    }
}

template <int TR>
struct S34Geom {
    static constexpr int SEG = S34_WAVES / TR;
    static constexpr int TC = 32 * SEG;
    static constexpr int PH = 2 * TR + 1, PW = 2 * TC + 1;
    static constexpr int NE = TC + 1;
    static constexpr int PP = PH * PW;
    static constexpr int SUB = PP * 16;
    static constexpr int PATCH = 4 * SUB;
    static constexpr int NSLOT = (PP * 8 + 255) / 256;
};

template <int NB>
struct S34Frag { f16x8 xh, xl, wh[NB], wl[NB]; };

template <int NB, int MB, int TR, bool HALF>
__global__ void __launch_bounds__(256, 2) conv3x3s2_pw_h1_kernel(Stem34Params p, int tiles_r, int tiles_c, int ntiles) {
    using G = S34Geom<TR>;
    extern __shared__ __attribute__((aligned(16))) unsigned char smem[];
    constexpr int SLAB = NB * 2 * 1024;
    constexpr int WPASS = S34_SLAB_STEPS * SLAB;
    constexpr int WPIECES = WPASS / 1024;
    constexpr int K2 = 2 * NB - (HALF ? 1 : 0);
    constexpr int NSLOT = G::NSLOT;
    const int tid = threadIdx.x, lane = tid & 63;
    const int wave = __builtin_amdgcn_readfirstlane(tid >> 6);
    const int l31 = lane & 31, lhi = lane >> 5;
    unsigned char* Pt = smem;
    unsigned char* Wb = smem + G::PATCH;
    float* Bs = reinterpret_cast<float*>(Wb + WPASS);
    float neg1 = -1.f;
    asm volatile("" : "+s"(neg1));
    const int passes = p.Cin / 16;

    auto dma_pass = [&](int ps) {
        if (p.abl & 16) return;
        const unsigned char* src = reinterpret_cast<const unsigned char*>(p.w3) + (size_t)ps * WPASS + lane * 16;
        unsigned char* dst = Wb;
#pragma unroll
        for (int u = 0; u < (WPIECES + S34_WAVES - 1) / S34_WAVES; ++u) {
            const int f = wave + u * S34_WAVES;
            if (f < WPIECES)
                __builtin_amdgcn_global_load_lds((const __attribute__((address_space(1))) void*)(src + f * 1024),
                                                 (__attribute__((address_space(3))) void*)(dst + f * 1024), 16, 0, 0);
        }
    };

    unsigned xmax = 0;
    u32x4 pre[NSLOT];
    unsigned pre_ok = 0;
    auto load_patch = [&](int im, int oh0, int ow0, int c0, int halves) {
        if (p.abl & 4) return;
        typedef __amdgpu_buffer_rsrc_t rsrc_t;
        const rsrc_t rx = __builtin_amdgcn_make_buffer_rsrc(const_cast<float*>(p.x + (size_t)im * p.H * p.W * p.xld + c0), 0, 0x7fffffff, 0x00020000);
        int stid = tid;
        asm volatile("" : "+v"(stid));
        pre_ok = 0;
#pragma unroll
        for (int i = 0; i < NSLOT; ++i) {
            const int q = stid + 256 * i;
            const int px = min(q >> 3, G::PP - 1), grp = (q & 7) ^ ((i & 1) << 2);
            const int row = px / G::PW, col = px - row * G::PW;
            const int ih = 2 * oh0 - 1 + row, iw = 2 * ow0 - 1 + col;
            if ((unsigned)ih < (unsigned)p.H && (unsigned)iw < (unsigned)p.W) pre_ok |= 1u << i;
            const unsigned gsel = grp < 4 * halves ? 16u * (unsigned)grp : 0u;
            const unsigned off = ((unsigned)min(max(ih, 0), p.H - 1) * (unsigned)p.W + (unsigned)min(max(iw, 0), p.W - 1)) * (unsigned)p.xld * 4u + gsel;
            pre[i] = __builtin_amdgcn_raw_buffer_load_b128(rx, (int)off, 0, 0);
        }
    };
    auto write_patch = [&](int half) {
        if (p.abl & 2) return;
        int stid = tid;
        asm volatile("" : "+v"(stid));
        const int tsel = ((stid >> 2) & 1) ^ half;
#pragma unroll
        for (int i = 0; i < NSLOT; ++i) {
            const int q = stid + 256 * i;
            if ((i & 1) != tsel || q >= G::PP * 8) continue;
            const int px = q >> 3, grp = q & 3;
            const int row = px / G::PW, col = px - row * G::PW;
            const f32x4 x4 = (pre_ok >> i) & 1u ? __builtin_bit_cast(f32x4, pre[i]) : f32x4{0.f, 0.f, 0.f, 0.f};
            f16x4 hi, lo;
            s34_split4(x4, neg1, hi, lo);
#pragma unroll
            for (int e = 0; e < 4; ++e) xmax = max(xmax, __float_as_uint(x4[e]) & 0x7fffffffu);
            const unsigned pos = (unsigned)(row * G::PW + ((col & 1) ? G::NE + (col >> 1) : (col >> 1)));
            const unsigned o = (unsigned)(grp >> 1) * G::SUB + pos * 16u + (unsigned)(grp & 1) * 8u;
            *reinterpret_cast<f16x4*>(Pt + o) = hi;
            *reinterpret_cast<f16x4*>(Pt + 2 * G::SUB + o) = lo;
        }
    };

    const int wr = wave % TR, wseg = wave / TR;
    const unsigned x_lane = (unsigned)lhi * G::SUB + (unsigned)((2 * wr) * G::PW + 32 * wseg + l31) * 16u;
    const unsigned w_lane = (unsigned)lane * 16u;
    auto read_frag = [&](S34Frag<NB>& f, int tap) {
        const int kh = tap / 3, kw = tap - 3 * kh;
        const unsigned a = x_lane + (unsigned)(kh * G::PW + (kw == 1 ? G::NE : kw == 2 ? 1 : 0)) * 16u;
        f.xh = *reinterpret_cast<const f16x8*>(Pt + a);
        f.xl = *reinterpret_cast<const f16x8*>(Pt + 2 * G::SUB + a);
        const unsigned char* wb = Wb + tap * SLAB + w_lane;
#pragma unroll
        for (int nb = 0; nb < NB; ++nb) {
            f.wh[nb] = *reinterpret_cast<const f16x8*>(wb + (2 * nb) * 1024);
            f.wl[nb] = *reinterpret_cast<const f16x8*>(wb + (2 * nb + 1) * 1024);
        }
    };

    f32x16 acc[NB];
    S34Frag<NB> fr[2];
    auto run_pass = [&]() {
        if (p.abl & 1) return;
        read_frag(fr[0], 0);
#pragma unroll
        for (int s = 0; s < S34_SLAB_STEPS; ++s) {
            S34Frag<NB>& cur = fr[s & 1];
            if (s + 1 < S34_SLAB_STEPS) read_frag(fr[(s + 1) & 1], s + 1);
#pragma unroll
            for (int nb = 0; nb < NB; ++nb) acc[nb] = __builtin_amdgcn_mfma_f32_32x32x16_f16(cur.wh[nb], cur.xh, acc[nb], 0, 0, 0);
#pragma unroll
            for (int nb = 0; nb < NB; ++nb) acc[nb] = __builtin_amdgcn_mfma_f32_32x32x16_f16(cur.wh[nb], cur.xl, acc[nb], 0, 0, 0);
#pragma unroll
            for (int nb = 0; nb < NB; ++nb) acc[nb] = __builtin_amdgcn_mfma_f32_32x32x16_f16(cur.wl[nb], cur.xh, acc[nb], 0, 0, 0);
        }
    };

    auto decode = [&](int v, int& im, int& oh0, int& ow0) {
        const int xcd = v & 7, jj = v >> 3, q = ntiles >> 3, rm = ntiles & 7;
        int t = (xcd < rm ? xcd * (q + 1) : rm * (q + 1) + (xcd - rm) * q) + jj;
        const int tc = t % tiles_c;
        t /= tiles_c;
        const int tr = t % tiles_r;
        im = t / tiles_r;
        oh0 = tr * TR;
        ow0 = tc * G::TC;
    };

    unsigned emax = 0;
    const uint16_t* w4 = p.w4;
    int v = blockIdx.x;
    if (v >= ntiles) return;
    for (int i = tid; i < NB * 32; i += 256) Bs[i] = p.b3[i];
    for (int i = tid; i < MB * 32; i += 256) Bs[NB * 32 + i] = i < p.N2 ? p.b4[i] : 0.f;
    int img, oh0, ow0;
    decode(v, img, oh0, ow0);
    if (p.abl >> 10) {
        const bool late = (p.abl & 512) ? ((int)blockIdx.x >= (int)gridDim.x / 2) : (((int)blockIdx.x >> 3) & 1);
        if (late) for (int i = 0; i < (p.abl >> 10); ++i) __builtin_amdgcn_s_sleep(127);
    }
    dma_pass(0);
    load_patch(img, oh0, ow0, 0, min(2, passes));
    write_patch(0);
    asm volatile("s_waitcnt vmcnt(0) lgkmcnt(0)\n\ts_barrier" ::: "memory");

#pragma unroll 1
    while (true) {
#pragma unroll
        for (int nb = 0; nb < NB; ++nb)
#pragma unroll
            for (int i = 0; i < 16; ++i) acc[nb][i] = 0.f;
        const int vn = v + (int)gridDim.x;
        int img_n = 0, oh_n = 0, ow_n = 0;
        if (vn < ntiles) decode(vn, img_n, oh_n, ow_n);
#pragma unroll 1
        for (int pass = 0; pass < passes; ++pass) {
            const bool last = pass + 1 == passes;
            const bool more = !last || vn < ntiles;
            const bool round_ends = (pass & 1) || last;
            if (round_ends && more) {
                if (!last) load_patch(img, oh0, ow0, (pass + 1) * 16, min(2, passes - pass - 1));
                else load_patch(img_n, oh_n, ow_n, 0, min(2, passes));
            }
            run_pass();
            if (last && !(p.abl & 8)) {
                f16x8 hb[K2], lb[K2];
                int lane_e = lane;
                asm volatile("" : "+v"(lane_e));
                const int lhie = lane_e >> 5, l31e = lane_e & 31;
#pragma unroll
                for (int nb = 0; nb < NB; ++nb) {
#pragma unroll
                    for (int r4 = 0; r4 < 4; ++r4) {
                        if (2 * nb + (r4 >> 1) >= K2) continue;
                        const f32x4 bv = *reinterpret_cast<const f32x4*>(Bs + 32 * nb + 8 * r4 + 4 * lhie);
                        f32x4 h;
#pragma unroll
                        for (int e = 0; e < 4; ++e) {
                            h[e] = fmaf(acc[nb][4 * r4 + e], p.w3_inv, bv[e]);
                            emax = max(emax, __float_as_uint(h[e]) & 0x7fffffffu);
                        }
                        if (p.act3 == ACT_RELU) {
#pragma unroll
                            for (int e = 0; e < 4; ++e) h[e] = fmaxf(h[e], 0.f);
                        } else if (p.act3 != ACT_NONE) {
#pragma unroll
                            for (int e = 0; e < 4; ++e) h[e] = rd_act(h[e], p.act3);
                        }
                        f16x4 hi, lo;
                        s34_split4(h, neg1, hi, lo);
                        const int j = 2 * nb + (r4 >> 1), e0 = 4 * (r4 & 1);
#pragma unroll
                        for (int e = 0; e < 4; ++e) {
                            hb[j][e0 + e] = hi[e];
                            lb[j][e0 + e] = lo[e];
                        }
                    }
                }
                const int oh = oh0 + wr;
                typedef __amdgpu_buffer_rsrc_t rsrc_t;
                const unsigned img_bytes = (unsigned)p.OH * (unsigned)p.OW * (unsigned)p.yld * 4u;
                const rsrc_t ry = __builtin_amdgcn_make_buffer_rsrc(p.y + (size_t)img * p.OH * p.OW * p.yld, 0, (int)img_bytes, 0x00020000);
                const unsigned rowbase = (unsigned)(min(oh, p.OH - 1) * p.OW) * (unsigned)p.yld * 4u;
                const int pw0 = ow0 + 32 * wseg + 4 * lhie;
                unsigned omax = 0;
#pragma unroll
                for (int mb = 0; mb < MB; ++mb) {
                    f32x16 a2;
#pragma unroll
                    for (int i = 0; i < 16; ++i) a2[i] = 0.f;
                    f16x8 wh[K2], wl[K2];
#pragma unroll
                    for (int j = 0; j < K2; ++j) {
                        wh[j] = *reinterpret_cast<const f16x8*>(w4 + ((size_t)(mb * K2 + j) * 2) * 512 + lane_e * 8);
                        wl[j] = *reinterpret_cast<const f16x8*>(w4 + ((size_t)(mb * K2 + j) * 2 + 1) * 512 + lane_e * 8);
                    }
#pragma unroll
                    for (int j = 0; j < K2; ++j) {
                        a2 = __builtin_amdgcn_mfma_f32_32x32x16_f16(hb[j], wh[j], a2, 0, 0, 0);
                        a2 = __builtin_amdgcn_mfma_f32_32x32x16_f16(lb[j], wh[j], a2, 0, 0, 0);
                        a2 = __builtin_amdgcn_mfma_f32_32x32x16_f16(hb[j], wl[j], a2, 0, 0, 0);
                    }
                    const int n = 32 * mb + l31e;
                    const float bv = Bs[NB * 32 + n];
                    const bool nok = n < p.N2 && oh < p.OH && !(p.abl & 32);
                    float o[16];
#pragma unroll
                    for (int i = 0; i < 16; ++i) {
                        o[i] = fmaf(a2[i], p.w4_inv, bv);
                        omax = max(omax, __float_as_uint(o[i]) & 0x7fffffffu);
                    }
                    if (p.act4 == ACT_RELU) {
#pragma unroll
                        for (int i = 0; i < 16; ++i) o[i] = fmaxf(o[i], 0.f);
                    } else if (p.act4 != ACT_NONE) {
#pragma unroll
                        for (int i = 0; i < 16; ++i) o[i] = rd_act(o[i], p.act4);
                    }
#pragma unroll
                    for (int i = 0; i < 16; ++i) {
                        const int pw = pw0 + (i & 3) + 8 * (i >> 2);
                        const unsigned off = (nok && pw < p.OW) ? rowbase + ((unsigned)pw * (unsigned)p.yld + (unsigned)n) * 4u : 0xfffffff0u;
                        __builtin_amdgcn_raw_buffer_store_b32(__float_as_uint(o[i]), ry, (int)off, 0, 2);
                    }
                }
                if (omax >= 0x7f800000u) emax = omax;
            }
            if (!more) break;
            asm volatile("s_barrier" ::: "memory");
            dma_pass(last ? 0 : pass + 1);
            write_patch(last ? 0 : ((pass + 1) & 1));
            asm volatile("s_waitcnt vmcnt(0) lgkmcnt(0)\n\ts_barrier" ::: "memory");
        }
        if (vn >= ntiles) break;
        v = vn; img = img_n; oh0 = oh_n; ow0 = ow_n;
    }
    if ((emax >= 0x477fe000u || xmax >= 0x477fe000u) && p.range_flag) rd_raise_flag(p.range_flag);
}

bool stem34_enabled() {
    static const bool on = [] { const char* e = getenv("RD_STEM34"); return e && e[0] == '1'; }();
    return on;
}
bool stem34_shape_ok(int cin, int n1, int n2) {
    return cin % 16 == 0 && cin >= 16 && cin <= 256 && n1 >= 8 && n1 <= 64 && n1 % 4 == 0 && n2 >= 8 && n2 <= 96 && n2 % 4 == 0 && !(n1 > 48 && n2 > 64);
}

static int wgs_per_cu() {
    static const int n = [] { const char* e = getenv("RD_STEM34_WGS"); return e ? atoi(e) : 2; }();
    return n;
}
template <int NB, int MB, int TR, bool HALF>
static void launch_stem34_t(const Stem34Params& p, hipStream_t s, int n_cu) {
    using G = S34Geom<TR>;
    const int tiles_r = (p.OH + TR - 1) / TR, tiles_c = (p.OW + G::TC - 1) / G::TC;
    const int ntiles = p.N * tiles_r * tiles_c;
    const size_t lds = (size_t)G::PATCH + (size_t)S34_SLAB_STEPS * NB * 2048 + (size_t)(NB + MB) * 32 * sizeof(float);
    static unsigned long long ok = 0;
    rd_allow_dynamic_lds((const void*)conv3x3s2_pw_h1_kernel<NB, MB, TR, HALF>, lds, ok);
    hipLaunchKernelGGL((conv3x3s2_pw_h1_kernel<NB, MB, TR, HALF>), dim3((unsigned)std::min(ntiles, wgs_per_cu() * n_cu)), dim3(256), lds, s, p, tiles_r, tiles_c, ntiles);
}

void launch_stem34(const Stem34Params& p_in, hipStream_t s) {
    if (p_in.N <= 0 || p_in.OH <= 0 || p_in.OW <= 0) return;
    static const int abl = [] { const char* e = getenv("RD_STEM34_ABL"); return e ? atoi(e) : 0; }();
    Stem34Params p = p_in;
    p.abl = abl;
    static const int n_cu = [] {
        int dev = 0, n = 256;
        (void)hipGetDevice(&dev);
        (void)hipDeviceGetAttribute(&n, hipDeviceAttributeMultiprocessorCount, dev);
        return n > 0 ? n : 256;
    }();
    const int nb = (p.N1 + 31) / 32, mb = (p.N2 + 31) / 32;
    auto covered = [&](int tr, int tc) { return (long)((p.OH + tr - 1) / tr * tr) * ((p.OW + tc - 1) / tc * tc); };
    static const int force_tr = [] { const char* e = getenv("RD_STEM34_TR"); return e ? atoi(e) : 0; }();
    const bool tr2 = force_tr ? force_tr == 2 : covered(2, 64) < covered(4, 32);
    const bool half = p.N1 <= 32 * nb - 16;
#define RD_S34_CASE(NBv, MBv, FULL)                                             \
    if (nb == NBv && mb == MBv) {                                               \
        if (half && tr2) launch_stem34_t<NBv, MBv, 2, true>(p, s, n_cu);        \
        else if (half) launch_stem34_t<NBv, MBv, 4, true>(p, s, n_cu);          \
        else if constexpr (FULL) {                                              \
            if (tr2) launch_stem34_t<NBv, MBv, 2, false>(p, s, n_cu);           \
            else launch_stem34_t<NBv, MBv, 4, false>(p, s, n_cu);               \
        }                                                                       \
        return;                                                                 \
    }
    RD_S34_CASE(1, 1, true) RD_S34_CASE(1, 2, true) RD_S34_CASE(1, 3, true) RD_S34_CASE(2, 1, true) RD_S34_CASE(2, 2, true) RD_S34_CASE(2, 3, false)
#undef RD_S34_CASE
}

static float s34_scale_exp(const float* w, size_t n, int& ex) {
    float mx = 0.f;
    for (size_t i = 0; i < n; ++i) mx = std::fmax(mx, std::fabs(w[i]));
    ex = 0;
    if (mx > 0.f && std::isfinite(mx)) {
        int x = 0;
        (void)std::frexp(mx, &x);
        ex = 14 - x;
        ex = ex > 100 ? 100 : ex < -100 ? -100 : ex;
    }
    return std::ldexp(1.f, -ex);
}
static void s34_put(float v, int ex, uint16_t& hb, uint16_t& lb) {
    const float vs = std::ldexp(v, ex);
    const _Float16 hh = (_Float16)vs;
    const _Float16 ll = (_Float16)(vs - (float)hh);
    __builtin_memcpy(&hb, &hh, 2);
    __builtin_memcpy(&lb, &ll, 2);
}

void prepare_stem34_weights(const float* w3, const float* w4, int Cin, int N1, int N2, std::vector<uint16_t>& img3, std::vector<uint16_t>& img4,
                            float inv[2]) {
    const int K = 9 * Cin, nb_n = (N1 + 31) / 32, mb_n = (N2 + 31) / 32, passes = Cin / 16, K2 = 2 * nb_n - (N1 <= 32 * nb_n - 16 ? 1 : 0);
    int ex3 = 0, ex4 = 0;
    inv[0] = s34_scale_exp(w3, (size_t)N1 * K, ex3);
    inv[1] = s34_scale_exp(w4, (size_t)N2 * N1, ex4);
    img3.assign((size_t)passes * 9 * nb_n * 2 * 512, 0);
    size_t slab = 0;
    for (int pass = 0; pass < passes; ++pass)
        for (int tap = 0; tap < 9; ++tap, ++slab)
            for (int nb = 0; nb < nb_n; ++nb)
                for (int lane = 0; lane < 64; ++lane) {
                    const int n = nb * 32 + (lane & 31);
                    if (n >= N1) continue;
                    for (int e = 0; e < 8; ++e) {
                        const int k = tap * Cin + pass * 16 + 8 * (lane >> 5) + e;
                        const size_t base = ((slab * nb_n + nb) * 2) * 512 + (size_t)lane * 8 + e;
                        s34_put(w3[(size_t)n * K + k], ex3, img3[base], img3[base + 512]);
                    }
                }
    img4.assign((size_t)mb_n * K2 * 2 * 512, 0);
    for (int mb = 0; mb < mb_n; ++mb)
        for (int j = 0; j < K2; ++j)
            for (int lane = 0; lane < 64; ++lane) {
                const int n = mb * 32 + (lane & 31);
                if (n >= N2) continue;
                for (int e = 0; e < 8; ++e) {
                    const int c = 16 * j + 8 * (e >> 2) + 4 * (lane >> 5) + (e & 3);
                    if (c >= N1) continue;
                    const size_t base = ((size_t)(mb * K2 + j) * 2) * 512 + (size_t)lane * 8 + e;
                    s34_put(w4[(size_t)n * N1 + c], ex4, img4[base], img4[base + 512]);
                }
            }
}

}
```

### rapiddoc_amd/csrc/kernels_stem_fused.hip

```cpp
#include <cmath>
#include <cstdlib>
#include <vector>

#include "rd_device.h"

namespace rd {

static constexpr int SF_TH = 8, SF_TW = 32;
static constexpr int SF_EH = SF_TH + 2, SF_EW = SF_TW + 2;
static constexpr int SF_AH = SF_TH + 1, SF_AW = SF_TW + 1;
static constexpr int SF_PH = 2 * SF_EH + 1, SF_PW = 2 * SF_EW + 1;
static constexpr int SF_PROW = 208;
static constexpr int SF_PATCH_FLOATS = SF_PH * SF_PROW + 16;
static constexpr int SF_NT = 512;

template <int C1>
struct SfGeom {
    static constexpr int CA = C1, NA = C1 / 2, CB = (NA + 7) / 8 * 8;
    static constexpr int K1 = 48, K2A = 4 * CA, K2B = 4 * CB;
    static constexpr int SE = CA + 4, SA = CB + 4;
    static_assert(((SE / 4) & 1) == 1 && ((SA / 4) & 1) == 1, "pixel strides must be 4 x odd floats");
    static constexpr int pad8(int k) { return ((k / 8) & 1) ? k : k + 8; }
    static constexpr int R1 = pad8(K1), R2A = pad8(K2A), R2B = pad8(K2B);
    static constexpr int W1_H = C1 * R1, W2A_H = NA * R2A, W2B_H = C1 * R2B;
    static constexpr int W_HALFS = 2 * (W1_H + W2A_H + W2B_H);
    static constexpr int IMG_HALFS = W_HALFS + 16;
    static constexpr int BIAS_FLOATS = C1 + NA + C1;
    static constexpr int E_FLOATS = (SF_EH * SF_EW + 31) / 32 * 32 * SE;
    static constexpr int A_FLOATS_RAW = (SF_AH * SF_AW + 31) / 32 * 32 * SA;
    static constexpr int A_FLOATS = A_FLOATS_RAW > SF_PATCH_FLOATS ? A_FLOATS_RAW : SF_PATCH_FLOATS;
    static constexpr size_t LDS_BYTES = (size_t)W_HALFS * 2 + (size_t)(BIAS_FLOATS + E_FLOATS + A_FLOATS) * 4 + 64;
    static constexpr int MB1 = (SF_EH * SF_EW + 31) / 32, NB1 = (C1 + 31) / 32;
    static constexpr int MB2 = (SF_AH * SF_AW + 31) / 32;
    static constexpr int MB3 = SF_TH * SF_TW / 32, NB3 = (C1 + 31) / 32;
    static_assert(NA <= 32 && MB3 == 8, "one N block for stem2a, one M block per wavefront for stem2b");
};

struct StemFusedParams {
    const float* x; int N, H, W, in_ch;
    const uint16_t* wimg;
    const float* bias;
    float* y; int yld;
    int H2, W2, tiles_x, tiles_y;
    unsigned* range_flag;
    const int32_t* line_tab;
    int dbg;
};

typedef _Float16 sf_f16x2 __attribute__((ext_vector_type(2)));
__device__ __forceinline__ void sf_split8(const f32x4 a, const f32x4 b, float neg1, f16x8& hi, f16x8& lo) {
#pragma unroll
    for (int e = 0; e < 4; e += 2) {
        const sf_f16x2 ha = __builtin_convertvector(f32x2{a[e], a[e + 1]}, sf_f16x2);
        const sf_f16x2 hb = __builtin_convertvector(f32x2{b[e], b[e + 1]}, sf_f16x2);
        hi[e] = ha[0];
        hi[e + 1] = ha[1];
        hi[4 + e] = hb[0];
        hi[4 + e + 1] = hb[1];
        lo[e] = (_Float16)__builtin_fmaf((float)ha[0], neg1, a[e]);
        lo[e + 1] = (_Float16)__builtin_fmaf((float)ha[1], neg1, a[e + 1]);
        lo[4 + e] = (_Float16)__builtin_fmaf((float)hb[0], neg1, b[e]);
        lo[4 + e + 1] = (_Float16)__builtin_fmaf((float)hb[1], neg1, b[e + 1]);
    }
}

template <int C1>
__global__ void __launch_bounds__(SF_NT, 2) stem_fused_kernel(StemFusedParams p) {
    using G = SfGeom<C1>;
    extern __shared__ __attribute__((aligned(16))) unsigned char lds[];
    _Float16* Wl = reinterpret_cast<_Float16*>(lds);
    float* Bs = reinterpret_cast<float*>(lds + (size_t)G::W_HALFS * 2);
    float* Es = Bs + ((G::BIAS_FLOATS + 3) & ~3);
    float* As = Es + G::E_FLOATS;
    const _Float16* W1h = Wl;
    const _Float16* W1l = Wl + G::W1_H;
    const _Float16* W2Ah = Wl + 2 * G::W1_H;
    const _Float16* W2Al = W2Ah + G::W2A_H;
    const _Float16* W2Bh = W2Ah + 2 * G::W2A_H;
    const _Float16* W2Bl = W2Bh + G::W2B_H;
    const float* b1 = Bs;
    const float* b2a = Bs + C1;
    const float* b2b = Bs + C1 + G::NA;

    const int tid = threadIdx.x, lane = tid & 63;
    const int wave = __builtin_amdgcn_readfirstlane(tid >> 6);
    const int l31 = lane & 31, lhi = lane >> 5;
    const float* scl = reinterpret_cast<const float*>(p.wimg + G::W_HALFS);
    const float inv1 = scl[0], inv2a = scl[1], inv2b = scl[2], sc1 = scl[3], sc2a = scl[4], sc2b = scl[5];
    float neg1 = -1.f;
    asm volatile("" : "+s"(neg1));

    for (int i = tid; i < G::W_HALFS / 8; i += SF_NT)
        reinterpret_cast<u32x4*>(Wl)[i] = reinterpret_cast<const u32x4*>(p.wimg)[i];
    for (int i = tid; i < G::BIAS_FLOATS; i += SF_NT) Bs[i] = p.bias[i];

    const int tiles_per_img = p.tiles_x * p.tiles_y, ntiles = p.N * tiles_per_img;
    constexpr int PATCH_ELEMS = SF_PH * SF_PW * 3;
    constexpr int PRE = (PATCH_ELEMS + SF_NT - 1) / SF_NT;
    float pre[PRE];
    auto tile_origin = [&](int t, int& n, int& ty0, int& tx0) {
        n = t / tiles_per_img;
        const int r = t - n * tiles_per_img;
        const int tyi = r / p.tiles_x;
        ty0 = tyi * SF_TH;
        tx0 = (r - tyi * p.tiles_x) * SF_TW;
    };
    int p_rc[PRE], p_lds[PRE], p_ci[PRE];
#pragma unroll
    for (int k = 0; k < PRE; ++k) {
        const int i = tid + k * SF_NT;
        const int row = i / (SF_PW * 3), rem = i - row * (SF_PW * 3);
        const int col = rem / 3, ci = rem - col * 3;
        p_rc[k] = i < PATCH_ELEMS ? (row << 16) | col : -1;
        p_lds[k] = row * SF_PROW + rem;
        p_ci[k] = (p.in_ch == 1 ? 0 : ci) * p.H * p.W;
    }
    auto load_patch = [&](int t) {
        int n, ty0, tx0;
        tile_origin(t, n, ty0, tx0);
        const int iy0 = 2 * ty0 - 1, ix0 = 2 * tx0 - 1;
        const float* img = p.x + (size_t)n * p.in_ch * p.H * p.W;
#pragma unroll
        for (int k = 0; k < PRE; ++k) {
            const int iy = min(max(iy0 + (p_rc[k] >> 16), 0), p.H - 1), ix = min(max(ix0 + (p_rc[k] & 0xffff), 0), p.W - 1);
            pre[k] = img[p_ci[k] + iy * p.W + ix];
        }
    };
    auto store_patch = [&](int ty0, int tx0) {
        const int iy0 = 2 * ty0 - 1, ix0 = 2 * tx0 - 1;
#pragma unroll
        for (int k = 0; k < PRE; ++k) {
            const int iy = iy0 + (p_rc[k] >> 16), ix = ix0 + (p_rc[k] & 0xffff);
            const bool ok = (unsigned)iy < (unsigned)p.H && (unsigned)ix < (unsigned)p.W;
            if (p_rc[k] >= 0) As[p_lds[k]] = ok ? pre[k] : 0.f;
        }
        if (tid < SF_PH) As[tid * SF_PROW + SF_PW * 3] = 0.f;
        if (tid >= 64 && tid < 80) As[SF_PH * SF_PROW + tid - 64] = 0.f;
    };

    unsigned emax = 0;
    int t = blockIdx.x;
    if (t < ntiles) load_patch(t);
    __syncthreads();
    for (; t < ntiles; t += gridDim.x) {
        int n, ty0, tx0;
        tile_origin(t, n, ty0, tx0);
        if (!(p.dbg & 16)) store_patch(ty0, tx0);
        __syncthreads();

        const int W2n = p.line_tab ? min(p.W2, p.line_tab[n * kLineTabStride + 1]) : p.W2;
        const bool inner = ty0 + SF_EH <= p.H2 && tx0 + SF_EW <= W2n;

        for (int mb = wave; mb < G::MB1 && !(p.dbg & 1); mb += 8) {
            const int m = min(mb * 32 + l31, SF_EH * SF_EW - 1);
            const int ey = m / SF_EW, ex = m - ey * SF_EW;
            f32x16 acc1[G::NB1], acc2[G::NB1];
#pragma unroll
            for (int nb = 0; nb < G::NB1; ++nb) {
                const float bv = b1[min(nb * 32 + l31, C1 - 1)] * sc1;
#pragma unroll
                for (int r = 0; r < 16; ++r) { acc1[nb][r] = bv; acc2[nb][r] = 0.f; }
            }
            const float* src0 = As + 2 * ey * SF_PROW + 2 * ex * 3 + 8 * lhi;
            f32x2 q[4];
            f16x8 wh[G::NB1], wl[G::NB1];
            auto fetch1 = [&](int kh) {
                const float* src = src0 + kh * SF_PROW;
#pragma unroll
                for (int i = 0; i < 4; ++i) q[i] = *reinterpret_cast<const f32x2*>(src + 2 * i);
#pragma unroll
                for (int nb = 0; nb < G::NB1; ++nb) {
                    const _Float16* wb = W1h + min(nb * 32 + l31, C1 - 1) * G::R1 + 8 * lhi + kh * 16;
                    wh[nb] = *reinterpret_cast<const f16x8*>(wb);
                    wl[nb] = *reinterpret_cast<const f16x8*>(wb + G::W1_H);
                }
            };
            fetch1(0);
#pragma unroll
            for (int kh = 0; kh < 3; ++kh) {
                const f32x4 v0 = f32x4{q[0][0], q[0][1], q[1][0], q[1][1]}, v1 = f32x4{q[2][0], q[2][1], q[3][0], q[3][1]};
                f16x8 bh[G::NB1], bl[G::NB1];
#pragma unroll
                for (int nb = 0; nb < G::NB1; ++nb) { bh[nb] = wh[nb]; bl[nb] = wl[nb]; }
                f16x8 ah, al;
                sf_split8(v0, v1, neg1, ah, al);
                __builtin_amdgcn_sched_barrier(0);
                if (kh + 1 < 3) fetch1(kh + 1);
                __builtin_amdgcn_sched_barrier(0);
#pragma unroll
                for (int nb = 0; nb < G::NB1; ++nb) {
                    acc1[nb] = __builtin_amdgcn_mfma_f32_32x32x16_f16(ah, bh[nb], acc1[nb], 0, 0, 0);
                    acc2[nb] = __builtin_amdgcn_mfma_f32_32x32x16_f16(ah, bl[nb], acc2[nb], 0, 0, 0);
                    acc2[nb] = __builtin_amdgcn_mfma_f32_32x32x16_f16(al, bh[nb], acc2[nb], 0, 0, 0);
                }
                __builtin_amdgcn_sched_barrier(0);
            }
#pragma unroll
            for (int nb = 0; nb < G::NB1; ++nb) {
                const int nn = nb * 32 + l31;
                float* dst = Es + (mb * 32 + 4 * lhi) * G::SE + nn;
                if (nn < C1) {
#pragma unroll
                    for (int r = 0; r < 16; ++r)
                        dst[((r & 3) + 8 * (r >> 2)) * G::SE] = fmaxf((acc1[nb][r] + acc2[nb][r]) * inv1, 0.f);
                }
            }
        }
        __syncthreads();
        const int vh = p.H2 - ty0, vw = W2n - tx0;
        if (!inner) {
            constexpr int C4 = C1 / 4;
            for (int i = tid; i < SF_EH * SF_EW * C4; i += SF_NT) {
                const int pix = i / C4, cg = i - pix * C4;
                const int cy = pix / SF_EW, cx = pix - cy * SF_EW;
                if (cy >= vh || cx >= vw) *reinterpret_cast<f32x4*>(Es + pix * G::SE + 4 * cg) = f32x4{0.f, 0.f, 0.f, 0.f};
            }
            __syncthreads();
        }

        for (int mb = wave; mb < G::MB2 && !(p.dbg & 2); mb += 8) {
            const int m = min(mb * 32 + l31, SF_AH * SF_AW - 1);
            const int ay = m / SF_AW, ax = m - ay * SF_AW;
            const int nrow = min(l31, G::NA - 1);
            const float bv = b2a[nrow] * sc2a;
            f32x16 acc1, acc2;
#pragma unroll
            for (int r = 0; r < 16; ++r) { acc1[r] = bv; acc2[r] = 0.f; }
            const float* src0 = Es + (ay * SF_EW + ax) * G::SE;
            const _Float16* wb = W2Ah + nrow * G::R2A + 8 * lhi;
            f32x4 nv0, nv1;
            f16x8 nbh, nbl;
            auto fetch2a = [&](int j) {
                constexpr int CAc = G::CA;
                const int t0 = (16 * j) / CAc, c0 = (16 * j) % CAc, t1 = (16 * j + 8) / CAc, c1 = (16 * j + 8) % CAc;
                const int o0 = ((t0 >> 1) * SF_EW + (t0 & 1)) * G::SE + c0, o1 = ((t1 >> 1) * SF_EW + (t1 & 1)) * G::SE + c1;
                const float* src = src0 + (lhi ? o1 : o0);
                nv0 = *reinterpret_cast<const f32x4*>(src);
                nv1 = *reinterpret_cast<const f32x4*>(src + 4);
                nbh = *reinterpret_cast<const f16x8*>(wb + 16 * j);
                nbl = *reinterpret_cast<const f16x8*>(wb + G::W2A_H + 16 * j);
            };
            fetch2a(0);
#pragma unroll
            for (int j = 0; j < G::K2A / 16; ++j) {
                const f32x4 v0 = nv0, v1 = nv1;
                const f16x8 bh = nbh, bl = nbl;
                f16x8 ah, al;
                sf_split8(v0, v1, neg1, ah, al);
                __builtin_amdgcn_sched_barrier(0);
                if (j + 1 < G::K2A / 16) fetch2a(j + 1);
                __builtin_amdgcn_sched_barrier(0);
                acc1 = __builtin_amdgcn_mfma_f32_32x32x16_f16(ah, bh, acc1, 0, 0, 0);
                acc2 = __builtin_amdgcn_mfma_f32_32x32x16_f16(ah, bl, acc2, 0, 0, 0);
                acc2 = __builtin_amdgcn_mfma_f32_32x32x16_f16(al, bh, acc2, 0, 0, 0);
                __builtin_amdgcn_sched_barrier(0);
            }
            float* dst = As + (mb * 32 + 4 * lhi) * G::SA + l31;
            const bool lane_on = l31 < G::CB;
            const bool real = l31 < G::NA;
            if (lane_on) {
#pragma unroll
                for (int r = 0; r < 16; ++r) {
                    const float v = (acc1[r] + acc2[r]) * inv2a;
                    dst[((r & 3) + 8 * (r >> 2)) * G::SA] = real ? fmaxf(v, 0.f) : 0.f;
                }
            }
        }
        {
            constexpr int C4 = C1 / 4;
            constexpr int FIRST = G::MB2 > 8 ? G::MB2 - 8 : 0, NTH = (8 - FIRST) * 64;
            if (wave >= FIRST && !(p.dbg & 4)) {
                for (int i = tid - FIRST * 64; i < SF_TH * SF_TW * C4; i += NTH) {
                    const int pix = i / C4, cg = i - pix * C4;
                    const int py = pix >> 5, px = pix & 31;
                    const int gy = ty0 + py, gx = tx0 + px;
                    if (gy >= p.H2 || gx >= p.W2) continue;
                    const float* e0 = Es + (py * SF_EW + px) * G::SE + 4 * cg;
                    const f32x4 a = *reinterpret_cast<const f32x4*>(e0), b = *reinterpret_cast<const f32x4*>(e0 + G::SE);
                    const f32x4 c = *reinterpret_cast<const f32x4*>(e0 + SF_EW * G::SE), d = *reinterpret_cast<const f32x4*>(e0 + (SF_EW + 1) * G::SE);
                    f32x4 o;
#pragma unroll
                    for (int k = 0; k < 4; ++k) o[k] = fmaxf(fmaxf(a[k], b[k]), fmaxf(c[k], d[k]));
                    emax = max(emax, __float_as_uint(o[0] + o[1] + o[2] + o[3]) & 0x7fffffffu);
                    __builtin_nontemporal_store(o, reinterpret_cast<f32x4*>(p.y + (((size_t)n * p.H2 + gy) * p.W2 + gx) * p.yld + 4 * cg));
                }
            }
        }
        __syncthreads();
        if (!inner) {
            constexpr int B4 = G::CB / 4;
            for (int i = tid; i < SF_AH * SF_AW * B4; i += SF_NT) {
                const int pix = i / B4, cg = i - pix * B4;
                const int ay = pix / SF_AW, ax = pix - ay * SF_AW;
                if (ay >= vh || ax >= vw) *reinterpret_cast<f32x4*>(As + pix * G::SA + 4 * cg) = f32x4{0.f, 0.f, 0.f, 0.f};
            }
            __syncthreads();
        }

        const int tn = t + (int)gridDim.x;
        if (tn < ntiles && !(p.dbg & 16)) load_patch(tn);

        if (!(p.dbg & 8)) {
            const int by = wave, bx = l31;
            f32x16 acc1[G::NB3], acc2[G::NB3];
#pragma unroll
            for (int nb = 0; nb < G::NB3; ++nb) {
                const float bv = b2b[min(nb * 32 + l31, C1 - 1)] * sc2b;
#pragma unroll
                for (int r = 0; r < 16; ++r) { acc1[nb][r] = bv; acc2[nb][r] = 0.f; }
            }
            const float* src0 = As + (by * SF_AW + bx) * G::SA;
            f32x4 nv0, nv1;
            f16x8 nwh[G::NB3], nwl[G::NB3];
            auto fetch2b = [&](int j) {
                constexpr int CBc = G::CB;
                const int t0 = (16 * j) / CBc, c0 = (16 * j) % CBc, t1 = (16 * j + 8) / CBc, c1 = (16 * j + 8) % CBc;
                const int o0 = ((t0 >> 1) * SF_AW + (t0 & 1)) * G::SA + c0, o1 = ((t1 >> 1) * SF_AW + (t1 & 1)) * G::SA + c1;
                const float* src = src0 + (lhi ? o1 : o0);
                nv0 = *reinterpret_cast<const f32x4*>(src);
                nv1 = *reinterpret_cast<const f32x4*>(src + 4);
#pragma unroll
                for (int nb = 0; nb < G::NB3; ++nb) {
                    const int nrow = min(nb * 32 + l31, C1 - 1);
                    nwh[nb] = *reinterpret_cast<const f16x8*>(W2Bh + nrow * G::R2B + 16 * j + 8 * lhi);
                    nwl[nb] = *reinterpret_cast<const f16x8*>(W2Bl + nrow * G::R2B + 16 * j + 8 * lhi);
                }
            };
            fetch2b(0);
#pragma unroll
            for (int j = 0; j < G::K2B / 16; ++j) {
                const f32x4 v0 = nv0, v1 = nv1;
                f16x8 bh[G::NB3], bl[G::NB3];
#pragma unroll
                for (int nb = 0; nb < G::NB3; ++nb) { bh[nb] = nwh[nb]; bl[nb] = nwl[nb]; }
                f16x8 ah, al;
                sf_split8(v0, v1, neg1, ah, al);
                __builtin_amdgcn_sched_barrier(0);
                if (j + 1 < G::K2B / 16) fetch2b(j + 1);
                __builtin_amdgcn_sched_barrier(0);
#pragma unroll
                for (int nb = 0; nb < G::NB3; ++nb) {
                    acc1[nb] = __builtin_amdgcn_mfma_f32_32x32x16_f16(ah, bh[nb], acc1[nb], 0, 0, 0);
                    acc2[nb] = __builtin_amdgcn_mfma_f32_32x32x16_f16(ah, bl[nb], acc2[nb], 0, 0, 0);
                    acc2[nb] = __builtin_amdgcn_mfma_f32_32x32x16_f16(al, bh[nb], acc2[nb], 0, 0, 0);
                }
                __builtin_amdgcn_sched_barrier(0);
            }
            __builtin_amdgcn_s_waitcnt(0x0F70);
            const int gy = ty0 + by;
            float* yrow = p.y + (((size_t)n * p.H2 + min(gy, p.H2 - 1)) * p.W2 + tx0 + 4 * lhi) * p.yld + C1;
#pragma unroll
            for (int nb = 0; nb < G::NB3; ++nb) {
                const int nn = nb * 32 + l31;
                if (inner) {
                    if (nn < C1) {
#pragma unroll
                        for (int r = 0; r < 16; ++r) {
                            const float v = (acc1[nb][r] + acc2[nb][r]) * inv2b;
                            emax = max(emax, __float_as_uint(v) & 0x7fffffffu);
                            __builtin_nontemporal_store(fmaxf(v, 0.f), &yrow[(size_t)((r & 3) + 8 * (r >> 2)) * p.yld + nn]);
                        }
                    }
                } else {
#pragma unroll
                    for (int r = 0; r < 16; ++r) {
                        const int off = (r & 3) + 8 * (r >> 2);
                        const float v = (acc1[nb][r] + acc2[nb][r]) * inv2b;
                        emax = max(emax, __float_as_uint(v) & 0x7fffffffu);
                        if (gy < p.H2 && tx0 + 4 * lhi + off < p.W2 && nn < C1)
                            yrow[(size_t)off * p.yld + nn] = tx0 + 4 * lhi + off < W2n ? fmaxf(v, 0.f) : 0.f;
                    }
                }
            }
        }
        __syncthreads();
    }
    if (emax >= 0x7f800000u && p.range_flag) rd_raise_flag(p.range_flag);
}

bool stem_fused_supported(int c1) { return c1 == 24 || c1 == 32 || c1 == 48; }

static int sf_scale_exp(const float* w, size_t n) {
    float mx = 0.f;
    for (size_t i = 0; i < n; ++i) mx = std::fmax(mx, std::fabs(w[i]));
    if (!(mx > 0.f) || !std::isfinite(mx)) return 0;
    int x = 0;
    (void)std::frexp(mx, &x);
    const int ex = 14 - x;
    return ex > 100 ? 100 : ex < -100 ? -100 : ex;
}

template <int C1>
static void sf_prepare(const float* w1, const float* w2a, const float* w2b, std::vector<uint16_t>& img) {
    using G = SfGeom<C1>;
    img.assign(G::IMG_HALFS, 0);
    const int ex[3] = {sf_scale_exp(w1, (size_t)27 * C1), sf_scale_exp(w2a, (size_t)G::NA * G::K2A), sf_scale_exp(w2b, (size_t)C1 * 4 * G::NA)};
    auto put = [&](size_t hi_at, size_t lo_at, float v, int e) {
        const float vs = std::ldexp(v, e);
        const _Float16 h = (_Float16)vs;
        const _Float16 l = (_Float16)(vs - (float)h);
        __builtin_memcpy(&img[hi_at], &h, 2);
        __builtin_memcpy(&img[lo_at], &l, 2);
    };
    for (int co = 0; co < C1; ++co)
        for (int kh = 0; kh < 3; ++kh)
            for (int j = 0; j < 9; ++j)
                put((size_t)co * G::R1 + kh * 16 + j, (size_t)G::W1_H + (size_t)co * G::R1 + kh * 16 + j, w1[(size_t)(kh * 9 + j) * C1 + co], ex[0]);
    const size_t o2a = 2 * (size_t)G::W1_H;
    for (int n = 0; n < G::NA; ++n)
        for (int k = 0; k < G::K2A; ++k)
            put(o2a + (size_t)n * G::R2A + k, o2a + G::W2A_H + (size_t)n * G::R2A + k, w2a[(size_t)n * G::K2A + k], ex[1]);
    const size_t o2b = o2a + 2 * (size_t)G::W2A_H;
    for (int n = 0; n < C1; ++n)
        for (int tap = 0; tap < 4; ++tap)
            for (int c = 0; c < G::NA; ++c)
                put(o2b + (size_t)n * G::R2B + tap * G::CB + c, o2b + G::W2B_H + (size_t)n * G::R2B + tap * G::CB + c,
                    w2b[(size_t)n * 4 * G::NA + tap * G::NA + c], ex[2]);
    float scl[6];
    for (int k = 0; k < 3; ++k) { scl[k] = std::ldexp(1.f, -ex[k]); scl[3 + k] = std::ldexp(1.f, ex[k]); }
    __builtin_memcpy(&img[G::W_HALFS], scl, sizeof(scl));
}
void prepare_stem_fused_weights(int c1, const float* w1, const float* w2a, const float* w2b, std::vector<uint16_t>& img) {
    if (c1 == 24) sf_prepare<24>(w1, w2a, w2b, img);
    else if (c1 == 32) sf_prepare<32>(w1, w2a, w2b, img);
    else sf_prepare<48>(w1, w2a, w2b, img);
}

template <int C1>
static void sf_launch(StemFusedParams& p, hipStream_t s, int n_cu) {
    static unsigned long long lds_ok = 0;
    rd_allow_dynamic_lds((const void*)stem_fused_kernel<C1>, SfGeom<C1>::LDS_BYTES, lds_ok);
    const int ntiles = p.N * p.tiles_x * p.tiles_y;
    hipLaunchKernelGGL(stem_fused_kernel<C1>, dim3(ntiles < n_cu ? ntiles : n_cu), dim3(SF_NT), SfGeom<C1>::LDS_BYTES, s, p);
}

void launch_stem_fused(int c1, const float* x, int N, int H, int W, int in_ch, const uint16_t* wimg, const float* bias, float* y, int yld,
                       unsigned* range_flag, hipStream_t s, const int32_t* line_tab) {
    static const int n_cu = [] {
        int dev = 0, n = 256;
        (void)hipGetDevice(&dev);
        (void)hipDeviceGetAttribute(&n, hipDeviceAttributeMultiprocessorCount, dev);
        return n > 0 ? n : 256;
    }();
    StemFusedParams p{};
    p.x = x; p.N = N; p.H = H; p.W = W; p.in_ch = in_ch;
    p.wimg = wimg; p.bias = bias; p.y = y; p.yld = yld;
    p.H2 = (H + 2 - 3) / 2 + 1;
    p.W2 = (W + 2 - 3) / 2 + 1;
    p.tiles_y = (p.H2 + SF_TH - 1) / SF_TH;
    p.tiles_x = (p.W2 + SF_TW - 1) / SF_TW;
    p.range_flag = range_flag;
    p.line_tab = line_tab;
    static const int dbg = [] { const char* e = getenv("RD_STEM_DBG"); return e ? atoi(e) : 0; }();
    p.dbg = dbg;
    if (c1 == 24) sf_launch<24>(p, s, n_cu);
    else if (c1 == 32) sf_launch<32>(p, s, n_cu);
    else sf_launch<48>(p, s, n_cu);
}

}
```

### rapiddoc_amd/csrc/models.cpp

```cpp
#include "engine.h"

namespace rd {

using G = Builder::ConvGeom;

static G geom(int k, int s = 1) {
    G g;
    g.kh = g.kw = k;
    g.sh = g.sw = s;
    g.pt = g.pl = g.pb = g.pr = (k - 1) / 2;
    return g;
}
static G geom_same_even(int k) {
    G g;
    g.kh = g.kw = k;
    g.pt = g.pl = (k - 1) / 2;
    g.pb = g.pr = (k - 1) - (k - 1) / 2;
    return g;
}

struct LcBlockCfg { int k, cin, cout, sh, sw; bool se; };
bool g_disable_fused_mixer = false;

static TView lc_stem(Builder& b, const std::string& p, const TView& x_nchw, int c1, int c2) {
    auto cw = [&](const char* n) { return p + "." + n + ".convolution.weight"; };
    auto bn = [&](const char* n) { return p + "." + n + ".normalization"; };
    (void)c1;
    TView cat = b.stem_front(cw("stem1"), bn("stem1"), cw("stem2a"), bn("stem2a"), cw("stem2b"), bn("stem2b"), x_nchw);
    TView s4 = b.stem_tail(cw("stem3"), bn("stem3"), cw("stem4"), bn("stem4"), cat, ACT_RELU, ACT_RELU);
    b.release(cat);
    (void)c2;
    return s4;
}

static TView lc_block(Builder& b, const std::string& p, const TView& x, const LcBlockCfg& c) {
    const bool rep = c.sh == 1 && c.sw == 1 && c.cin == c.cout;
    G g = geom(c.k);
    g.sh = c.sh;
    g.sw = c.sw;
    TView t;
    Builder::GapOut gap;
    Builder::GapOut* gp = c.se ? &gap : nullptr;
    const bool fuse_dw = rep && !c.se && c.k == 3 && mixer_fused_supported(c.cin) && !g_disable_fused_mixer && b.mixer_takes_dw(p, c.cin);
    if (fuse_dw) {
        const std::string key = Builder::dw_key(p + ".token_conv.weight", "");
        return b.mixer_fused(p, x, nullptr, &key);
    }
    if (rep) t = b.dwconv(p + ".token_conv.weight", p + ".token_conv.bias", "", x, g, ACT_NONE, nullptr, nullptr, gp);
    else t = b.dwconv(p + ".token_conv.convolution.weight", "", p + ".token_conv.normalization", x, g, ACT_NONE, nullptr, nullptr, gp);
    TView gate;
    bool has_gate = false;
    if (c.se) {
        const std::string s = p + ".token_squeeze_excitation.convolutions.";
        gate = b.se_gate(s + "0.weight", s + "0.bias", s + "2.weight", s + "2.bias", t, ACT_HSIG, &gap);
        has_gate = true;
    }
    if (rep && mixer_fused_supported(c.cin) && !g_disable_fused_mixer) {
        TView o = b.mixer_fused(p, t, has_gate ? &gate : nullptr);
        if (has_gate) b.release(gate);
        b.release(t);
        return o;
    }
    if (has_gate) {
        b.scale(t, gate, 0.f, t);
        b.release(gate);
    }
    TView m = b.conv(p + ".channel_conv1.convolution.weight", "", p + ".channel_conv1.normalization", t, geom(1), ACT_GELU);
    TView o = b.conv(p + ".channel_conv2.convolution.weight", "", p + ".channel_conv2.normalization", m, geom(1), ACT_NONE,
                     nullptr, rep ? &t : nullptr);
    b.release(m);
    b.release(t);
    return o;
}

static const std::vector<std::vector<LcBlockCfg>> kDetSmall = {
    {{3, 48, 48, 1, 1, true}, {3, 48, 48, 1, 1, false}},
    {{3, 48, 96, 2, 2, false}, {3, 96, 96, 1, 1, true}, {3, 96, 96, 1, 1, false}},
    {{3, 96, 192, 2, 2, false}, {3, 192, 192, 1, 1, true}, {3, 192, 192, 1, 1, false}, {3, 192, 192, 1, 1, true},
     {3, 192, 192, 1, 1, false}},
    {{3, 192, 384, 2, 2, false}, {3, 384, 384, 1, 1, true}, {3, 384, 384, 1, 1, false}},
};
static const std::vector<std::vector<LcBlockCfg>> kRecSmall = {
    {{3, 96, 96, 1, 1, true}},
    {{3, 96, 96, 1, 1, false}, {3, 96, 96, 1, 1, false}},
    {{3, 96, 192, 2, 1, false}, {3, 192, 192, 1, 1, true}, {3, 192, 192, 1, 1, false}, {3, 192, 192, 1, 1, true},
     {3, 192, 192, 1, 1, false}, {3, 192, 192, 1, 1, true}, {3, 192, 192, 1, 1, false}},
    {{3, 192, 384, 2, 1, false}, {3, 384, 384, 1, 1, true}, {3, 384, 384, 1, 1, false}},
};

static std::vector<TView> lcnetv4(Builder& b, const TView& x_nchw, const std::vector<std::vector<LcBlockCfg>>& cfg,
                                  int c1, int c2, bool keep_all) {
    const std::string enc = "backbone.encoder";
    TView h = lc_stem(b, enc + ".convolution", x_nchw, c1, c2);
    std::vector<TView> feats;
    for (size_t si = 0; si < cfg.size(); ++si) {
        for (size_t bi = 0; bi < cfg[si].size(); ++bi) {
            TView o = lc_block(b, enc + ".blocks." + std::to_string(si) + ".blocks." + std::to_string(bi), h, cfg[si][bi]);
            const bool is_feat = !feats.empty() && feats.back().buf == h.buf;
            if (!is_feat) b.release(h);
            h = o;
        }
        if (keep_all || si + 1 == cfg.size()) feats.push_back(h);
    }
    return feats;
}

void build_ppocrv6_det(Builder& b, int B, int H, int W) {
    RD_CHECK(H % 32 == 0 && W % 32 == 0 && H >= 32 && W >= 32, "det input H, W must be multiples of 32");
    TView x = b.external(0, B, H, W, 3);
    TView out = b.external(1, B, H, W, 1);
    std::vector<TView> f = lcnetv4(b, x, kDetSmall, 24, 48, true);

    std::vector<TView> fused(4);
    for (int i = 0; i < 4; ++i) {
        const std::string p = "neck.insert_conv." + std::to_string(i);
        TView y = b.conv(p + ".in_conv.weight", "", "", f[i], geom(1), ACT_NONE);
        b.release(f[i]);
        const std::string s = p + ".squeeze_excitation_block.";
        TView gate = b.se_gate(s + "conv1.weight", s + "conv1.bias", s + "conv2.weight", s + "conv2.bias", y, ACT_HSIG_PADDLE);
        b.scale(y, gate, 1.f, y);
        b.release(gate);
        fused[i] = y;
    }
    for (int i = 2; i >= 0; --i) b.upsample(fused[i + 1], fused[i], 2, true);
    TView cat = b.alloc(B, H / 4, W / 4, 96);
    for (int i = 0; i < 4; ++i) {
        const std::string p = "neck.input_conv." + std::to_string(i);
        TView d = b.dwconv(p + ".depthwise_convolution.weight", p + ".depthwise_convolution.bias", "", fused[i], geom(7), ACT_NONE);
        b.release(fused[i]);
        TView z = b.conv(p + ".pointwise_convolution.weight", "", "", d, geom(1), ACT_NONE);
        b.release(d);
        const std::string s = p + ".squeeze_excitation_module.";
        TView gate = b.se_gate(s + "conv1.weight", s + "conv1.bias", s + "conv2.weight", s + "conv2.bias", z, ACT_HSIG_PADDLE);
        TView slot = b.slice(cat, 24 * (3 - i), 24);
        if (i == 0) {
            b.scale(z, gate, 1.f, slot);
        } else {
            b.scale(z, gate, 1.f, z);
            b.upsample(z, slot, 1 << i, false);
        }
        b.release(gate);
        b.release(z);
    }
    TView c = b.conv("head.conv_down.convolution.weight", "", "head.conv_down.norm", cat, geom(3), ACT_RELU);
    b.release(cat);
    if (b.deconv_pair_to_prob("head.conv_up.convolution.weight", "head.conv_up.convolution.bias", "head.conv_up.norm", "head.conv_final.weight",
                              "head.conv_final.bias", c, out)) {
        b.release(c);
    } else {
        TView u = b.deconv2x2("head.conv_up.convolution.weight", "head.conv_up.convolution.bias", "head.conv_up.norm", c, ACT_RELU);
        b.release(c);
        b.deconv2x2("head.conv_final.weight", "head.conv_final.bias", "", u, ACT_SIGMOID, &out);
        b.release(u);
    }
}

void build_ppocrv6_rec(Builder& b, int B, int H, int W, int flags) {
    const bool tail_only = (flags & REC_STAGE_TAIL) != 0, backbone_only = (flags & REC_STAGE_BACKBONE) != 0;
    RD_CHECK(!(tail_only && backbone_only), "rec: choose one stage");
    const std::string e = "head.encoder";
    auto cw = [&](int i) { return e + ".conv_block." + std::to_string(i) + ".convolution.weight"; };
    auto cbn = [&](int i) { return e + ".conv_block." + std::to_string(i) + ".normalization"; };
    TView pooled, seg, tokinfo;
    int T, n_seq = B;
    if (tail_only) {
        RD_CHECK((flags & ~REC_STAGE_TAIL) == 0, "rec tail: fused CTC only");
        RD_CHECK(B >= 1 && H >= 1 && H < 32768 && W >= B, "rec tail: B lines, H = longest line (tokens), W = all tokens");
        pooled = b.external(0, 1, 1, W, b.weight_dim(cw(0), 1));
        seg = b.external(4, B, 1, 1, 2);
        tokinfo = b.external(5, 1, 1, W, 1);
        T = H;
    } else {
        RD_CHECK(H == 48, "rec input height must be 48");
        RD_CHECK(W >= 16, "rec input width must be >= 16");
        TView x = b.external(0, B, H, W, 3);
        if (flags & REC_LINE_WIDTHS) {
            RD_CHECK(backbone_only, "rec: per-line widths belong to the backbone stage");
            b.set_line_table(b.external(2, B, 1, 1, kLineTabStride));
        }
        std::vector<TView> f = lcnetv4(b, x, kRecSmall, 48, 96, false);
        if (backbone_only) {
            RD_CHECK((flags & ~(REC_STAGE_BACKBONE | REC_LINE_WIDTHS)) == 0, "rec backbone stage takes no other flag");
            TView out = b.external(1, B, 1, (f[0].w - 2) / 2 + 1, f[0].c);
            b.avgpool3x2(f[0], &out);
            b.release(f[0]);
            return;
        }
        pooled = b.avgpool3x2(f[0]);
        b.release(f[0]);
        T = pooled.w;
        RD_CHECK(pooled.h == 1, "rec: pooled height");
    }
    const TView* ti = tail_only ? &tokinfo : nullptr;
    const TView* sg = tail_only ? &seg : nullptr;

    TView res = b.conv(cw(0), "", cbn(0), pooled, geom(1), ACT_SILU);
    TView h = b.conv(cw(1), "", cbn(1), pooled, geom(1), ACT_SILU);
    b.release(pooled);
    G g17;
    g17.kh = 1;
    g17.kw = b.weight_dim(cw(2), 3);
    g17.pl = g17.pr = g17.kw / 2;
    TView t = b.dwconv(cw(2), "", cbn(2), h, g17, ACT_SILU, nullptr, &h, nullptr, ti);
    b.release(h);
    const int C = t.c, heads = 8, hd = C / heads;
    int depth = 0;
    while (b.has_weight(e + ".svtr_block." + std::to_string(depth) + ".layer_norm1.weight")) ++depth;
    for (int d = 0; d < depth; ++d) {
        const std::string p = e + ".svtr_block." + std::to_string(d);
        TView y = b.layernorm(p + ".layer_norm1", t, 1e-6f);
        TView qkv = b.linear(p + ".self_attn.qkv", y, ACT_NONE);
        b.release(y);
        TView a = b.attention(qkv, n_seq, T, heads, hd, sg);
        b.release(qkv);
        TView t2 = b.linear(p + ".self_attn.projection", a, ACT_NONE, nullptr, &t);
        b.release(a);
        b.release(t);
        TView y2 = b.layernorm(p + ".layer_norm2", t2, 1e-6f);
        TView m = b.linear(p + ".mlp.fc1", y2, ACT_SILU);
        b.release(y2);
        t = b.linear(p + ".mlp.fc2", m, ACT_NONE, nullptr, &t2);
        b.release(m);
        b.release(t2);
    }
    TView n = b.layernorm(e + ".norm", t, 1e-6f);
    b.release(t);
    TView seq = b.add(n, res);
    b.release(n);
    b.release(res);

    const int ncls = b.weight_dim("head.head.weight", 0);
    TView idx = tail_only ? b.external(1, 1, 1, W, 1) : b.external(1, B, 1, T, 1);
    TView prob = tail_only ? b.external(2, 1, 1, W, 1) : b.external(2, B, 1, T, 1);
    const bool want_full = (flags & (REC_WANT_SOFTMAX | REC_WANT_LOGITS)) != 0;
    if ((flags & REC_UNFUSED_CTC) || want_full) {
        if (flags & REC_WANT_LOGITS) {
            TView lg = b.external(3, B, 1, T, ncls);
            b.linear("head.head", seq, ACT_NONE, &lg);
            b.ctc_stats(lg, idx, prob);
        } else {
            TView lg = b.linear("head.head", seq, ACT_NONE);
            if (flags & REC_WANT_SOFTMAX) {
                TView sm = b.external(3, B, 1, T, ncls);
                b.softmax_rows(lg, sm, &idx, &prob);
            } else {
                b.ctc_stats(lg, idx, prob);
            }
            b.release(lg);
        }
    } else {
        b.ctc_head("head.head", seq, idx, prob);
    }
    b.release(seq);
}

struct HgStageCfg { int cin, mid, cout, blocks; bool down, light; int k, layers; };
static const HgStageCfg kB4Det[4] = {
    {48, 48, 128, 1, false, false, 3, 6},
    {128, 96, 512, 1, true, false, 3, 6},
    {512, 192, 1024, 3, true, true, 5, 6},
    {1024, 384, 2048, 1, true, true, 5, 6},
};

static const HgStageCfg kB6Formula[4] = {
    {96, 96, 192, 2, false, false, 3, 6},
    {192, 192, 512, 3, true, false, 3, 6},
    {512, 384, 1024, 6, true, true, 5, 6},
    {1024, 768, 2048, 3, true, true, 5, 6},
};

template <typename Emit>
static void build_pphgnetv2(Builder& b, const TView& x, const HgStageCfg (&cfg)[4], const std::string& pre, Emit emit) {
    const int B = x.n;
    auto cw = [&](const std::string& p) { return pre + p + ".conv.weight"; };
    auto bn = [&](const std::string& p) { return pre + p + ".bn"; };
    TView cat = b.stem_front(cw("stem.stem1"), bn("stem.stem1"), cw("stem.stem2a"), bn("stem.stem2a"), cw("stem.stem2b"),
                             bn("stem.stem2b"), x);

    TView cur, cur_cat;
    auto new_cat = [&](int n, int h, int w, const HgStageCfg& c, int cin) { return b.alloc(n, h, w, cin + c.layers * c.mid); };
    {
        const HgStageCfg& c = cfg[0];
        RD_CHECK(!c.down, "PPHGNetV2: the first stage does not downsample");
        const int s3h = (cat.h + 2 - 3) / 2 + 1, s3w = (cat.w + 2 - 3) / 2 + 1;
        cur_cat = new_cat(B, s3h, s3w, c, c.cin);
        cur = b.slice(cur_cat, 0, c.cin);
        b.stem_tail(cw("stem.stem3"), bn("stem.stem3"), cw("stem.stem4"), bn("stem.stem4"), cat, ACT_RELU, ACT_RELU, &cur);
        b.release(cat);
    }
    for (int si = 0; si < 4; ++si) {
        const HgStageCfg& c = cfg[si];
        const std::string sp = "stages." + std::to_string(si);
        RD_CHECK(si == 0 || c.down, "PPHGNetV2: stages 2-4 downsample");
        if (c.down) {
            const int oh = (cur.h + 2 - 3) / 2 + 1, ow = (cur.w + 2 - 3) / 2 + 1;
            TView ncat = new_cat(B, oh, ow, c, c.cin);
            TView nin = b.slice(ncat, 0, c.cin);
            b.dwconv(cw(sp + ".downsample"), "", bn(sp + ".downsample"), cur, geom(3, 2), ACT_NONE, &nin);
            b.release(cur_cat);
            cur_cat = ncat;
            cur = nin;
        }
        for (int bi = 0; bi < c.blocks; ++bi) {
            const std::string bp = sp + ".blocks." + std::to_string(bi);
            const int cin = bi == 0 ? c.cin : c.cout;
            TView prev = cur;
            for (int li = 0; li < c.layers; ++li) {
                const std::string lp = bp + ".layers." + std::to_string(li);
                TView slot = b.slice(cur_cat, cin + li * c.mid, c.mid);
                if (c.light) {
                    TView t = b.conv(cw(lp + ".conv1"), "", bn(lp + ".conv1"), prev, geom(1), ACT_NONE);
                    b.dwconv(cw(lp + ".conv2"), "", bn(lp + ".conv2"), t, geom(c.k), ACT_RELU, &slot);
                    b.release(t);
                } else {
                    b.conv(cw(lp), "", bn(lp), prev, geom(c.k), ACT_RELU, &slot);
                }
                prev = slot;
            }
            TView full = b.slice(cur_cat, 0, cin + c.layers * c.mid);
            TView sq = b.conv(cw(bp + ".aggregation_squeeze_conv"), "", bn(bp + ".aggregation_squeeze_conv"), full, geom(1), ACT_RELU);
            const bool last_block = bi + 1 == c.blocks;
            TView ncat, nout;
            if (!last_block) {
                ncat = new_cat(B, cur.h, cur.w, c, c.cout);
                nout = b.slice(ncat, 0, c.cout);
            } else {
                ncat = b.alloc(B, cur.h, cur.w, c.cout);
                nout = ncat;
            }
            const bool identity = bi > 0;
            b.conv(cw(bp + ".aggregation_excitation_conv"), "", bn(bp + ".aggregation_excitation_conv"), sq, geom(1), ACT_RELU,
                   &nout, identity ? &cur : nullptr);
            b.release(sq);
            b.release(cur_cat);
            cur_cat = ncat;
            cur = nout;
        }
        emit(si, cur);
    }
    b.release(cur_cat);
}

void build_pphgnetv2_b4(Builder& b, int B, int H, int W) {
    RD_CHECK(H % 32 == 0 && W % 32 == 0 && H >= 64 && W >= 64, "backbone input H, W must be multiples of 32 (>= 64)");
    TView x = b.external(0, B, H, W, 3);
    build_pphgnetv2(b, x, kB4Det, "", [&](int si, const TView& v) {
        TView o = b.external(1 + si, B, v.h, v.w, v.c);
        b.to_nchw(v, o);
    });
}

void build_pphgnetv2_b6_formula(Builder& b, int B, int H, int W, int flags) {
    RD_CHECK(H % 32 == 0 && W % 32 == 0 && H >= 64 && W >= 64, "formula encoder input H, W must be multiples of 32 (>= 64)");
    TView x = b.external(0, B, H, W, (flags & 1) ? 1 : 3);
    build_pphgnetv2(b, x, kB6Formula, "backbone.pphgnet_b6.", [&](int si, const TView& v) {
        if (si != 3) return;
        TView o = b.external(1, B, v.h, v.w, v.c);
        b.copy(v, o);
    });
}

}
```

### rapiddoc_amd/csrc/rd_kernels.h

```cpp
#pragma once
#include <hip/hip_runtime.h>
#include <cstdint>
#include <cstdlib>
#include <vector>

namespace rd {

inline void rd_allow_dynamic_lds(const void* kernel, size_t bytes, unsigned long long& mask) {
    int dev = 0;
    (void)hipGetDevice(&dev);
    const unsigned long long bit = 1ull << (dev & 63);
    if (!(mask & bit)) {
        (void)hipFuncSetAttribute(kernel, hipFuncAttributeMaxDynamicSharedMemorySize, (int)bytes);
        mask |= bit;
    }
}

inline int rd_cu_budget(int n_cu) {
    static const int env = [] { const char* e = std::getenv("RD_PERSISTENT_CUS"); return e ? std::atoi(e) : 0; }();
    return env > 0 && env < n_cu ? env : n_cu;
}

enum Act : int { ACT_NONE = 0, ACT_RELU = 1, ACT_GELU = 2, ACT_SILU = 3, ACT_SIGMOID = 4, ACT_HSIG = 5, ACT_HSIG_PADDLE = 6 };
enum OutMode : int { OUT_NHWC = 0, OUT_DECONV2X2 = 1 };

struct ConvParams {
    const float* x; int xld;
    int N, H, W, Cin;
    const float* w;
    const uint16_t* wh;
    const uint16_t* wl;
    const float* bias;
    float* y; int yld;
    int OH, OW, Cout;
    int KH, KW, SH, SW, PT, PL;
    const float* res; int rld;
    const float* ascale;
    const float* ln_g; const float* ln_b;
    int act, out_mode;
    int M, K, Ng;
    unsigned* range_flag = nullptr;
    const uint16_t* w1 = nullptr;
    float w1_inv = 0.f;
    int allow_skinny = 0;
    const uint16_t* w3 = nullptr;
    float w3_inv = 0.f;
    int fast_epi = 1;
};
void launch_conv_igemm(const ConvParams& p, hipStream_t s);
bool skinny_gemm_applies(int M, int K);
bool gemm_h3_dma_applies(const ConvParams& p);
bool gemm_h3_dma_uses16(const ConvParams& p);
void launch_gemm_h3_dma(const ConvParams& p, hipStream_t s);
bool gemm_h1_shape_ok(int K, int cout);
bool gemm_h1_applies(const ConvParams& p);
void launch_gemm_h1(const ConvParams& p, hipStream_t s);
float prepare_gemm_h1_weights(const float* w, int N, int K, std::vector<uint16_t>& img);
void launch_conv_igemm_h3(const ConvParams& p, hipStream_t s);
void launch_msdeform_attn(const float* value, const int32_t* shapes, const int32_t* start, const float* loc, const float* attn, float* out, int B,
                          int S, int H, int D, int Q, int L, int P, hipStream_t s);
void launch_topk_rows(const float* scores, int rows, int n, int k, float* out_vals, int32_t* out_idx, hipStream_t s);
struct Stem34Params {
    const float* x; int xld;
    int N, H, W, Cin;
    float* y; int yld;
    int OH, OW, N1, N2;
    const uint16_t* w3; float w3_inv; const float* b3;
    const uint16_t* w4; float w4_inv; const float* b4;
    int act3, act4;
    unsigned* range_flag = nullptr;
    int abl = 0;
};
bool stem34_shape_ok(int cin, int n1, int n2);
bool stem34_enabled();
void launch_stem34(const Stem34Params& p, hipStream_t s);
void prepare_stem34_weights(const float* w3, const float* w4, int Cin, int N1, int N2, std::vector<uint16_t>& img3, std::vector<uint16_t>& img4,
                            float inv[2]);
bool conv3x3_h1_shape_ok(int kh, int kw, int cin, int cout);
bool conv3x3_h1_applies(const ConvParams& p);
void launch_conv3x3_h1(const ConvParams& p, hipStream_t s);
float prepare_conv3x3_h1_weights(const float* w, int N, int Cin, std::vector<uint16_t>& img);
bool conv_direct_h3_supported(const ConvParams& p);
bool conv_direct_h3_applies(const ConvParams& p);
void launch_conv_direct_h3(const ConvParams& p, hipStream_t s);
bool conv_stream_h3_supported(const ConvParams& p);
bool conv_stream_h3_applies(const ConvParams& p);
void launch_conv_stream_h3(const ConvParams& p, hipStream_t s);
inline bool conv_stream_h3_shape_ok(int kh, int kw, int cin, int cout) {
    return cin % 4 == 0 && cin <= 64 && kh * kw * ((cin + 15) / 16 * 16) <= 256 && cout <= 96;
}
const char* conv_igemm_config_name(const ConvParams& p);

struct StemParams {
    const float* x;
    int N, H, W, in_ch;
    const float* w;
    const float* bias;
    float* y; int yld; int OH, OW, Cout;
    int act;
};
void launch_stem_conv3x3s2(const StemParams& p, hipStream_t s);

bool stem_fused_supported(int c1);
void prepare_stem_fused_weights(int c1, const float* w1_stem_layout, const float* w2a_folded, const float* w2b_folded, std::vector<uint16_t>& img);
void launch_stem_fused(int c1, const float* x, int N, int H, int W, int in_ch, const uint16_t* wimg, const float* bias, float* y, int yld,
                       unsigned* range_flag, hipStream_t s, const int32_t* line_tab = nullptr);

constexpr int kLineTabStride = 4;

struct DwParams {
    const float* x; int xld;
    int N, H, W, C;
    const float* w;
    const float* bias;
    float* y; int yld;
    int OH, OW, KH, KW, SH, SW, PT, PL;
    int act;
    const float* res; int rld;
    float* gap_partial;
    int gap_chunks;
    const int32_t* tokinfo = nullptr;
    const int32_t* line_w = nullptr; int line_w_stride = 0;
    int dbg = 0;
};
void launch_dwconv(const DwParams& p, hipStream_t s);
int dwconv_gap_chunks(const DwParams& p);
bool dwconv_lds_applies(const DwParams& p);
int dwconv_lds_gap_chunks(const DwParams& p);
void launch_dwconv_lds(const DwParams& p, hipStream_t s);
bool dwconv_kxk_lds_applies(const DwParams& p);
void launch_dwconv_kxk_lds(const DwParams& p, hipStream_t s);

void launch_maxpool2x2s1(const float* x, int xld, float* y, int yld, int N, int H, int W, int C, hipStream_t s);
void launch_avgpool3x2(const float* x, int xld, float* y, int yld, int N, int H, int W, int C, hipStream_t s, const int32_t* line_tab = nullptr);
void launch_mask_cols(float* y, int yld, int N, int H, int W, int C, const int32_t* line_w, int stride, hipStream_t s);

void launch_gap_partial(const float* x, int xld, int N, int HW, int C, float* partial, int chunks, hipStream_t s);
struct SeFcParams {
    const float* partial; int chunks; int N, C, Cr; float inv_hw;
    const float* w1; const float* b1;
    const float* w2; const float* b2;
    int gate;
    float* scale;
    const int32_t* line_w = nullptr; int line_w_stride = 0; int H = 0;
};
void launch_se_fc(const SeFcParams& p, hipStream_t s);
bool det_head_tail_supported(int cin, int cmid, int cout);
void launch_det_head_tail(const float* x, int xld, int N, int H, int W, const float* w1, const float* b1, const float* w2, const float* b2,
                          float* y, hipStream_t s);
void launch_scale_channels(const float* x, int xld, float* y, int yld, const float* scale, float alpha,
                           int N, int HW, int C, hipStream_t s);

void launch_upsample(const float* x, int xld, float* y, int yld, int N, int H, int W, int C, int f, int accumulate,
                     hipStream_t s);

void launch_layernorm(const float* x, int xld, float* y, int yld, const float* g, const float* b, int M, int C,
                      float eps, hipStream_t s);
int attention_h3_max_t();
bool attention_h3_applies(int T, int hd);
void launch_attention_h3(const float* qkv, float* o, int B, int T, int heads, int hd, float scale, hipStream_t s, const int32_t* seg);
void launch_attention(const float* qkv, float* o, int B, int T, int heads, int hd, float scale, hipStream_t s, const int32_t* seg = nullptr);

void launch_add(const float* a, int ald, const float* b, int bld, float* y, int yld, int M, int C, hipStream_t s);

void launch_rowmax_softmax(const float* logits, int ld, int M, int C, int32_t* idx, float* prob, hipStream_t s);
void launch_row_softmax(const float* logits, int ld, float* out, int M, int C, hipStream_t s, int32_t* idx = nullptr, float* prob = nullptr);
struct CtcParams {
    const float* x; int xld;
    const float* w;
    const float* bias;
    int M, K, C;
    float* part;
    int nsplit;
    int32_t* idx; float* prob;
    const uint16_t* wh = nullptr; const uint16_t* wl = nullptr;
    unsigned* range_flag = nullptr;
};
void launch_ctc_head(const CtcParams& p, hipStream_t s);
int ctc_head_nsplit(int M, int C, bool split_fp16);

void launch_nhwc_to_nchw(const float* x, int xld, float* y, int N, int H, int W, int C, hipStream_t s);
void launch_nchw_to_nhwc(const float* x, float* y, int yld, int N, int C, int H, int W, hipStream_t s);

struct PreprocParams {
    const uint8_t* src; int H, W;
    float* dst; int OH, OW;
    float mean[3], inv_std[3]; float scale;
    int interp;
    int swap_rb;
    int batch = 1;
    size_t src_stride = 0, dst_stride = 0;
};
void launch_preproc_resize_norm(const PreprocParams& p, hipStream_t s);

struct CropDesc {
    int32_t page;
    int32_t out_w;
    float crop_w, crop_h;
    float m[9];
    int32_t rot90;
    int32_t pad_;
};
struct CropBatchParams {
    const uint8_t* pages; int H, W; size_t page_stride;
    const CropDesc* descs; int n;
    float* dst; int OH, OWp;
    float mean[3], inv_std[3]; float scale; int swap_rb;
};
void launch_crop_resize_norm_batch(const CropBatchParams& p, hipStream_t s);

struct LineCropDesc {
    int32_t page;
    int32_t out_w;
    int32_t crop_w, crop_h;
    int32_t rot90;
    int32_t scratch_off;
    double m[9];
};
struct LineCropParams {
    const uint8_t* pages; int H, W; size_t page_stride;
    const LineCropDesc* descs; int n;
    uint8_t* scratch; long max_crop_pixels;
    float* dst; int OH, OWp;
    int swap_rb;
};
int launch_line_crops(const LineCropParams& p, hipStream_t s);
int launch_line_warp(const LineCropParams& p, hipStream_t s);
int launch_line_resize_norm(const LineCropParams& p, hipStream_t s);
int launch_db_scores(const float* prob, int B, int H, int W, const void* cand, const int32_t* n_cand, int max_cand, double* scores, hipStream_t s);
size_t db_boxes_workspace_bytes(int B, int H, int max_runs, int max_cand);
int launch_db_boxes(const float* prob, int B, int H, int W, const int32_t* src_hw_dev, float thresh, float box_thresh, float unclip_ratio,
                    int dilate, int max_cand, int max_runs, void* ws, size_t ws_bytes, void* out_boxes, int max_out, int32_t* n_out_dev,
                    hipStream_t s);
int launch_ctc_collapse(const int32_t* idx, const float* prob, int B, int T, const int32_t* seg, const uint8_t* ctab, int max_len, int n_classes,
                        uint8_t* out, int row_bytes, uint16_t* kept_cols, float* kept_conf, hipStream_t s);

}

namespace rd {
void split_weights_h3(const float* w, int rows, int K, std::vector<uint16_t>& hi, std::vector<uint16_t>& lo);
struct MixerParams {
    const float* x; int xld;
    float* y; int yld;
    int M, HW, C;
    const float* gate;
    const float* w1; const float* b1; const float* w2; const float* b2;
    const uint16_t* w1h = nullptr; const uint16_t* w1l = nullptr; const uint16_t* w2h = nullptr; const uint16_t* w2l = nullptr;
    unsigned* range_flag = nullptr;
    int dbg = 0;
    float ws_inv1 = 1.f, ws_inv2 = 1.f;
    bool ws_pf = false;
    const float* dw_w = nullptr; const float* dw_b = nullptr;
    int dwH = 0, dwW = 0;
    const int32_t* dw_line_w = nullptr; int dw_line_w_stride = 0;
};
bool mixer_fused_supported(int C);
bool mixer_res_fuses_dw(int C);
void launch_mixer_fused_h3(const MixerParams& p, hipStream_t s);
void prepare_mixer_weights_h3(const float* w1, const float* w2, int C, std::vector<uint16_t>& w1h, std::vector<uint16_t>& w1l,
                              std::vector<uint16_t>& w2h, std::vector<uint16_t>& w2l);
void launch_mixer_fused(const MixerParams& p, hipStream_t s);
bool mixer_ws_supported(int C);
bool mixer_ws_preferred(int C);
void prepare_mixer_weights_ws(const float* w1, const float* w2, int C, std::vector<uint16_t>& img, float inv[2]);
bool mixer_ws_prefetch();
void launch_mixer_fused_ws(const MixerParams& p, hipStream_t s);
void launch_mixer_debug(const MixerParams& p, int variant, hipStream_t s);
bool mixer_res_supported(int C);
void prepare_mixer_weights_res(const float* w1, const float* w2, int C, std::vector<uint16_t>& img, float inv[2]);
void launch_mixer_fused_res(const MixerParams& p, hipStream_t s);
}
```

Baseline: 349.0.

## Emit stem front output as pre-split fp16 hi/lo planes for stem tail

When the fused stem-tail route applies, the fused stem-front kernel now writes its concatenated output as split fp16 hi and lo planes instead of fp32. The stem34 kernel then reads these planes directly into LDS, skipping its own fp32-to-fp16x2 split during the patch load. This moves the split work to the producer and changes the intermediate layout to the same byte size. It adds an extra range check for the fp16 overflow in the producer, and the producer now does scattered 2-element stores, which may cost more than the old nontemporal fp32 stores.

```diff
diff --git a/rapiddoc_amd/csrc/api.cpp b/rapiddoc_amd/csrc/api.cpp
--- a/rapiddoc_amd/csrc/api.cpp
+++ b/rapiddoc_amd/csrc/api.cpp
@@ -535,8 +535,8 @@
     return iters > 0 ? ms / iters : 0.f;
 }
 
-float rd_debug_stem34(int N, int H, int W, int Cin, int xld, int N1, int N2, int yld, int act3, int act4, int iters, float* x, float* w3, float* b3,
-                      float* w4, float* b4, float* y, unsigned* range_flag) {
+static float debug_stem34(bool x_planes, int N, int H, int W, int Cin, int xld, int N1, int N2, int yld, int act3, int act4, int iters, float* x,
+                          float* w3, float* b3, float* w4, float* b4, float* y, unsigned* range_flag) {
     if (!rd::stem34_shape_ok(Cin, N1, N2)) return -1.f;
     std::vector<float> h3((size_t)N1 * 9 * Cin), h4((size_t)N2 * N1), hb3((size_t)((N1 + 31) / 32) * 32, 0.f);
     if (hipMemcpy(h3.data(), w3, h3.size() * 4, hipMemcpyDeviceToHost) != hipSuccess) return -1.f;
@@ -556,6 +556,7 @@
     p.w3 = (const uint16_t*)d3; p.w3_inv = inv[0]; p.b3 = (const float*)db3;
     p.w4 = (const uint16_t*)d4; p.w4_inv = inv[1]; p.b4 = b4;
     p.act3 = act3; p.act4 = act4; p.range_flag = range_flag;
+    p.x_planes = x_planes;
     hipEvent_t e0, e1;
     (void)hipEventCreate(&e0); (void)hipEventCreate(&e1);
     rd::launch_stem34(p, nullptr);
@@ -567,6 +568,41 @@
     (void)hipEventElapsedTime(&ms, e0, e1);
     (void)hipEventDestroy(e0); (void)hipEventDestroy(e1);
     (void)hipFree(d3); (void)hipFree(d4); (void)hipFree(db3);
+    return iters > 0 ? ms / iters : 0.f;
+}
+float rd_debug_stem34(int N, int H, int W, int Cin, int xld, int N1, int N2, int yld, int act3, int act4, int iters, float* x, float* w3, float* b3,
+                      float* w4, float* b4, float* y, unsigned* range_flag) {
+    return debug_stem34(false, N, H, W, Cin, xld, N1, N2, yld, act3, act4, iters, x, w3, b3, w4, b4, y, range_flag);
+}
+float rd_debug_stem34_planes(int N, int H, int W, int Cin, int xld, int N1, int N2, int yld, int act3, int act4, int iters, float* x, float* w3,
+                             float* b3, float* w4, float* b4, float* y, unsigned* range_flag) {
+    return debug_stem34(true, N, H, W, Cin, xld, N1, N2, yld, act3, act4, iters, x, w3, b3, w4, b4, y, range_flag);
+}
+
+float rd_debug_stem_fused(int c1, int N, int H, int W, int in_ch, int yld, int planes, int iters, const float* x, const float* w1, const float* w2a,
+                          const float* w2b, const float* bias, float* y, unsigned* range_flag, const int32_t* line_tab) {
+    if (!rd::stem_fused_supported(c1)) return -1.f;
+    std::vector<uint16_t> img;
+    rd::prepare_stem_fused_weights(c1, w1, w2a, w2b, img);
+    const size_t nb = (size_t)(c1 + c1 / 2 + c1) * 4;
+    void *dimg = nullptr, *db = nullptr;
+    if (hipMalloc(&dimg, img.size() * 2) != hipSuccess || hipMalloc(&db, nb) != hipSuccess) return -1.f;
+    (void)hipMemcpy(dimg, img.data(), img.size() * 2, hipMemcpyHostToDevice);
+    (void)hipMemcpy(db, bias, nb, hipMemcpyHostToDevice);
+    auto go = [&] {
+        rd::launch_stem_fused(c1, x, N, H, W, in_ch, (const uint16_t*)dimg, (const float*)db, y, yld, range_flag, nullptr, line_tab, planes != 0);
+    };
+    hipEvent_t e0, e1;
+    (void)hipEventCreate(&e0); (void)hipEventCreate(&e1);
+    go();
+    (void)hipEventRecord(e0, nullptr);
+    for (int i = 0; i < iters; ++i) go();
+    (void)hipEventRecord(e1, nullptr);
+    (void)hipEventSynchronize(e1);
+    float ms = 0.f;
+    (void)hipEventElapsedTime(&ms, e0, e1);
+    (void)hipEventDestroy(e0); (void)hipEventDestroy(e1);
+    (void)hipFree(dimg); (void)hipFree(db);
     return iters > 0 ? ms / iters : 0.f;
 }
 
diff --git a/rapiddoc_amd/csrc/engine.cpp b/rapiddoc_amd/csrc/engine.cpp
--- a/rapiddoc_amd/csrc/engine.cpp
+++ b/rapiddoc_amd/csrc/engine.cpp
@@ -709,12 +709,13 @@
 }
 
 TView Builder::stem_front(const std::string& w1, const std::string& bn1, const std::string& w2a, const std::string& bn2a,
-                          const std::string& w2b, const std::string& bn2b, const TView& xin) {
+                          const std::string& w2b, const std::string& bn2b, const TView& xin, bool planes) {
     const int c1 = weight_dim(w1, 0);
     ConvGeom g2;
     g2.kh = g2.kw = 2;
     g2.pb = g2.pr = 1;
     const std::string fkey = w1 + "|" + bn1 + "|stemfront";
+    planes_buf_ = -1;
     const bool off = std::getenv("RD_STEM_FUSED") && std::getenv("RD_STEM_FUSED")[0] == '0';
     const bool fused = planning() && !off && (h3_ || mixer_h3_) && pb_->has(fkey + "#img");
     if (!fused) {
@@ -759,7 +760,7 @@
     const uint16_t* img = reinterpret_cast<const uint16_t*>(pb_->ptr(fkey + "#img"));
     const float* bias = pb_->ptr(fkey + "#bias");
     OpRecord r;
-    r.name = w1 + ":front";
+    r.name = w1 + (planes ? ":front_planes" : ":front");
     r.kind = "stem_fused";
     r.cfg = "C" + std::to_string(c1);
     r.shape = "N" + std::to_string(xin.n) + "_" + std::to_string(oh) + "x" + std::to_string(ow);
@@ -770,12 +771,25 @@
     unsigned* flag = range_flag_;
     const bool has_lt = has_lt_;
     const TView ltv = lt_;
-    r.run = [xv, yv, img, bias, c1, flag, has_lt, ltv](const Plan& pl, const RunCtx& c) {
+    r.run = [xv, yv, img, bias, c1, flag, has_lt, ltv, planes](const Plan& pl, const RunCtx& c) {
         launch_stem_fused(c1, pl.vptr(xv, c), xv.n, xv.h, xv.w, xv.c, img, bias, pl.vptr(yv, c), pl.ld(yv), flag, c.stream,
-                          has_lt ? reinterpret_cast<const int32_t*>(pl.vptr(ltv, c)) : nullptr);
-    };
-    emit(std::move(r));
+                          has_lt ? reinterpret_cast<const int32_t*>(pl.vptr(ltv, c)) : nullptr, planes);
+    };
+    emit(std::move(r));
+    planes_buf_ = planes ? cat.buf : -1;
     return cat;
+}
+
+bool Builder::stem34_route(const std::string& fkey, int h, int w, int ld, int n2, int out_ld, int out_coff) const {
+    const int oh = out_dim(h, 3, 2, 1, 1), ow = out_dim(w, 3, 2, 1, 1);
+    return planning() && stem34_enabled() && (h3_ || mixer_h3_) && pb_->has(fkey + "#w3") && ld % 4 == 0 && (size_t)h * w * ld < ((size_t)1 << 30) &&
+           (!out_ld || (out_ld % 4 == 0 && out_coff % 4 == 0)) && (size_t)oh * ow * (out_ld ? out_ld : n2) < ((size_t)1 << 29);
+}
+
+bool Builder::stem_tail_takes_planes(const std::string& w3, const std::string& bn3, const std::string& w4, const std::string& bn4,
+                                     const TView& x_nchw, int out_ld, int out_coff) const {
+    const std::string fkey = w3 + "|" + bn3 + "|" + w4 + "|" + bn4 + "|stemtail";
+    return stem34_route(fkey, out_dim(x_nchw.h, 3, 2, 1, 1), out_dim(x_nchw.w, 3, 2, 1, 1), weight_dim(w3, 1), weight_dim(w4, 0), out_ld, out_coff);
 }
 
 TView Builder::stem_tail(const std::string& w3, const std::string& bn3, const std::string& w4, const std::string& bn4, const TView& x, int act3,
@@ -788,9 +802,10 @@
     ConvGeom g1;
     const std::string fkey = w3 + "|" + bn3 + "|" + w4 + "|" + bn4 + "|stemtail";
     const int oh = out_dim(x.h, 3, 2, 1, 1), ow = out_dim(x.w, 3, 2, 1, 1);
-    const bool fused = planning() && stem34_enabled() && (h3_ || mixer_h3_) && pb_->has(fkey + "#w3") && plan_->ld(x) % 4 == 0 &&
-                       (size_t)x.h * x.w * plan_->ld(x) < ((size_t)1 << 30) && (!out || (plan_->ld(*out) % 4 == 0 && out->coff % 4 == 0)) &&
-                       (size_t)oh * ow * (out ? plan_->ld(*out) : n2) < ((size_t)1 << 29);
+    const bool fused = stem34_route(fkey, x.h, x.w, plan_->ld(x), n2, out ? plan_->ld(*out) : 0, out ? out->coff : 0);
+    const bool x_planes = planning() && planes_buf_ >= 0 && x.buf == planes_buf_;
+    planes_buf_ = -1;
+    RD_CHECK(fused || !x_planes, "stem_tail: split-plane input but no fused route: " + w3);
     if (!fused) {
         TView s3 = conv(w3, "", bn3, x, g3, act3);
         TView s4 = conv(w4, "", bn4, s3, g1, act4, out);
@@ -831,8 +846,9 @@
     p.w4_inv = pb_->host_ptr(fkey + "#inv")[1];
     p.act3 = act3; p.act4 = act4;
     p.range_flag = range_flag_;
-    OpRecord r;
-    r.name = w3 + ":tail";
+    p.x_planes = x_planes;
+    OpRecord r;
+    r.name = w3 + (x_planes ? ":tail_planes" : ":tail");
     r.kind = "stem_tail";
     r.cfg = "C" + std::to_string(cin) + "_" + std::to_string(n1) + "_" + std::to_string(n2);
     r.shape = "M" + std::to_string(x.n * oh * ow) + "_K" + std::to_string(9 * cin) + "_N" + std::to_string(n1) + "_N" + std::to_string(n2);
diff --git a/rapiddoc_amd/csrc/engine.h b/rapiddoc_amd/csrc/engine.h
--- a/rapiddoc_amd/csrc/engine.h
+++ b/rapiddoc_amd/csrc/engine.h
@@ -165,7 +165,9 @@
                     const TView* out = nullptr);
     TView stem3x3s2(const std::string& wname, const std::string& bn, const TView& x_nchw, int act);
     TView stem_front(const std::string& w1, const std::string& bn1, const std::string& w2a, const std::string& bn2a,
-                     const std::string& w2b, const std::string& bn2b, const TView& x_nchw);
+                     const std::string& w2b, const std::string& bn2b, const TView& x_nchw, bool planes = false);
+    bool stem_tail_takes_planes(const std::string& w3, const std::string& bn3, const std::string& w4, const std::string& bn4,
+                                const TView& x_nchw, int out_ld = 0, int out_coff = 0) const;
     TView stem_tail(const std::string& w3, const std::string& bn3, const std::string& w4, const std::string& bn4, const TView& x, int act3,
                     int act4, const TView* out = nullptr);
     struct GapOut { TView partial; int chunks = 0; };
@@ -193,6 +195,7 @@
 
    private:
     void emit(OpRecord&& r) { plan_->ops.push_back(std::move(r)); }
+    bool stem34_route(const std::string& fkey, int h, int w, int ld, int n2, int out_ld, int out_coff) const;
     std::vector<float> bn_scale_shift(const std::string& bn, int c, std::vector<float>& shift) const;
     Mode mode_;
     bool h3_ = false;
@@ -205,6 +208,7 @@
     std::vector<Block> blocks_;
     TView lt_;
     bool has_lt_ = false;
+    int planes_buf_ = -1;
 };
 
 class Engine {
diff --git a/rapiddoc_amd/csrc/kernels_stem34.hip b/rapiddoc_amd/csrc/kernels_stem34.hip
--- a/rapiddoc_amd/csrc/kernels_stem34.hip
+++ b/rapiddoc_amd/csrc/kernels_stem34.hip
@@ -38,7 +38,7 @@
 template <int NB>
 struct S34Frag { f16x8 xh, xl, wh[NB], wl[NB]; };
 
-template <int NB, int MB, int TR, bool HALF>
+template <int NB, int MB, int TR, bool HALF, bool XP>
 __global__ void __launch_bounds__(256, 2) conv3x3s2_pw_h1_kernel(Stem34Params p, int tiles_r, int tiles_c, int ntiles) {
     using G = S34Geom<TR>;
     extern __shared__ __attribute__((aligned(16))) unsigned char smem[];
@@ -76,7 +76,7 @@
     auto load_patch = [&](int im, int oh0, int ow0, int c0, int halves) {
         if (p.abl & 4) return;
         typedef __amdgpu_buffer_rsrc_t rsrc_t;
-        const rsrc_t rx = __builtin_amdgcn_make_buffer_rsrc(const_cast<float*>(p.x + (size_t)im * p.H * p.W * p.xld + c0), 0, 0x7fffffff, 0x00020000);
+        const rsrc_t rx = __builtin_amdgcn_make_buffer_rsrc(const_cast<float*>(p.x + (size_t)im * p.H * p.W * p.xld + (XP ? 0 : c0)), 0, 0x7fffffff, 0x00020000);
         int stid = tid;
         asm volatile("" : "+v"(stid));
         pre_ok = 0;
@@ -87,7 +87,9 @@
             const int row = px / G::PW, col = px - row * G::PW;
             const int ih = 2 * oh0 - 1 + row, iw = 2 * ow0 - 1 + col;
             if ((unsigned)ih < (unsigned)p.H && (unsigned)iw < (unsigned)p.W) pre_ok |= 1u << i;
-            const unsigned gsel = grp < 4 * halves ? 16u * (unsigned)grp : 0u;
+            const unsigned gsel = grp >= 4 * halves ? 0u
+                                  : XP ? (unsigned)((grp >> 1) & 1) * (unsigned)p.Cin * 2u + (unsigned)(c0 + 16 * (grp >> 2) + 8 * (grp & 1)) * 2u
+                                       : 16u * (unsigned)grp;
             const unsigned off = ((unsigned)min(max(ih, 0), p.H - 1) * (unsigned)p.W + (unsigned)min(max(iw, 0), p.W - 1)) * (unsigned)p.xld * 4u + gsel;
             pre[i] = __builtin_amdgcn_raw_buffer_load_b128(rx, (int)off, 0, 0);
         }
@@ -103,6 +105,12 @@
             if ((i & 1) != tsel || q >= G::PP * 8) continue;
             const int px = q >> 3, grp = q & 3;
             const int row = px / G::PW, col = px - row * G::PW;
+            if constexpr (XP) {
+                const unsigned pos = (unsigned)(row * G::PW + ((col & 1) ? G::NE + (col >> 1) : (col >> 1)));
+                const u32x4 v = (pre_ok >> i) & 1u ? pre[i] : u32x4{0u, 0u, 0u, 0u};
+                *reinterpret_cast<u32x4*>(Pt + (unsigned)(grp >> 1) * 2 * G::SUB + (unsigned)(grp & 1) * G::SUB + pos * 16u) = v;
+                continue;
+            }
             const f32x4 x4 = (pre_ok >> i) & 1u ? __builtin_bit_cast(f32x4, pre[i]) : f32x4{0.f, 0.f, 0.f, 0.f};
             f16x4 hi, lo;
             s34_split4(x4, neg1, hi, lo);
@@ -288,7 +296,7 @@
         if (vn >= ntiles) break;
         v = vn; img = img_n; oh0 = oh_n; ow0 = ow_n;
     }
-    if ((emax >= 0x477fe000u || xmax >= 0x477fe000u) && p.range_flag) rd_raise_flag(p.range_flag);
+    if ((emax >= 0x477fe000u || (!XP && xmax >= 0x477fe000u)) && p.range_flag) rd_raise_flag(p.range_flag);
 }
 
 bool stem34_enabled() {
@@ -303,15 +311,20 @@
     static const int n = [] { const char* e = getenv("RD_STEM34_WGS"); return e ? atoi(e) : 2; }();
     return n;
 }
-template <int NB, int MB, int TR, bool HALF>
-static void launch_stem34_t(const Stem34Params& p, hipStream_t s, int n_cu) {
+template <int NB, int MB, int TR, bool HALF, bool XP>
+static void launch_stem34_x(const Stem34Params& p, hipStream_t s, int n_cu) {
     using G = S34Geom<TR>;
     const int tiles_r = (p.OH + TR - 1) / TR, tiles_c = (p.OW + G::TC - 1) / G::TC;
     const int ntiles = p.N * tiles_r * tiles_c;
     const size_t lds = (size_t)G::PATCH + (size_t)S34_SLAB_STEPS * NB * 2048 + (size_t)(NB + MB) * 32 * sizeof(float);
     static unsigned long long ok = 0;
-    rd_allow_dynamic_lds((const void*)conv3x3s2_pw_h1_kernel<NB, MB, TR, HALF>, lds, ok);
-    hipLaunchKernelGGL((conv3x3s2_pw_h1_kernel<NB, MB, TR, HALF>), dim3((unsigned)std::min(ntiles, wgs_per_cu() * n_cu)), dim3(256), lds, s, p, tiles_r, tiles_c, ntiles);
+    rd_allow_dynamic_lds((const void*)conv3x3s2_pw_h1_kernel<NB, MB, TR, HALF, XP>, lds, ok);
+    hipLaunchKernelGGL((conv3x3s2_pw_h1_kernel<NB, MB, TR, HALF, XP>), dim3((unsigned)std::min(ntiles, wgs_per_cu() * n_cu)), dim3(256), lds, s, p, tiles_r, tiles_c, ntiles);
+}
+template <int NB, int MB, int TR, bool HALF>
+static void launch_stem34_t(const Stem34Params& p, hipStream_t s, int n_cu) {
+    if (p.x_planes) launch_stem34_x<NB, MB, TR, HALF, true>(p, s, n_cu);
+    else launch_stem34_x<NB, MB, TR, HALF, false>(p, s, n_cu);
 }
 
 void launch_stem34(const Stem34Params& p_in, hipStream_t s) {
diff --git a/rapiddoc_amd/csrc/kernels_stem_fused.hip b/rapiddoc_amd/csrc/kernels_stem_fused.hip
--- a/rapiddoc_amd/csrc/kernels_stem_fused.hip
+++ b/rapiddoc_amd/csrc/kernels_stem_fused.hip
@@ -64,7 +64,18 @@
     }
 }
 
-template <int C1>
+__device__ __forceinline__ void sf_split4(const f32x4 v, float neg1, f16x4& hi, f16x4& lo) {
+#pragma unroll
+    for (int e = 0; e < 4; e += 2) {
+        const sf_f16x2 h = __builtin_convertvector(f32x2{v[e], v[e + 1]}, sf_f16x2);
+        hi[e] = h[0];
+        hi[e + 1] = h[1];
+        lo[e] = (_Float16)__builtin_fmaf((float)h[0], neg1, v[e]);
+        lo[e + 1] = (_Float16)__builtin_fmaf((float)h[1], neg1, v[e + 1]);
+    }
+}
+
+template <int C1, bool PLANES>
 __global__ void __launch_bounds__(SF_NT, 2) stem_fused_kernel(StemFusedParams p) {
     using G = SfGeom<C1>;
     extern __shared__ __attribute__((aligned(16))) unsigned char lds[];
@@ -139,6 +150,8 @@
     };
 
     unsigned emax = 0;
+    unsigned smax = 0;
+    _Float16* yh = reinterpret_cast<_Float16*>(p.y);
     int t = blockIdx.x;
     if (t < ntiles) load_patch(t);
     __syncthreads();
@@ -282,7 +295,18 @@
 #pragma unroll
                     for (int k = 0; k < 4; ++k) o[k] = fmaxf(fmaxf(a[k], b[k]), fmaxf(c[k], d[k]));
                     emax = max(emax, __float_as_uint(o[0] + o[1] + o[2] + o[3]) & 0x7fffffffu);
-                    __builtin_nontemporal_store(o, reinterpret_cast<f32x4*>(p.y + (((size_t)n * p.H2 + gy) * p.W2 + gx) * p.yld + 4 * cg));
+                    const size_t pix_at = ((size_t)n * p.H2 + gy) * p.W2 + gx;
+                    if constexpr (PLANES) {
+                        f16x4 hi, lo;
+                        sf_split4(o, neg1, hi, lo);
+#pragma unroll
+                        for (int k = 0; k < 4; ++k) smax = max(smax, __float_as_uint(o[k]) & 0x7fffffffu);
+                        _Float16* dst = yh + pix_at * 2 * p.yld + 4 * cg;
+                        *reinterpret_cast<f16x4*>(dst) = hi;
+                        *reinterpret_cast<f16x4*>(dst + 2 * C1) = lo;
+                    } else {
+                        __builtin_nontemporal_store(o, reinterpret_cast<f32x4*>(p.y + pix_at * p.yld + 4 * cg));
+                    }
                 }
             }
         }
@@ -348,7 +372,45 @@
             }
             __builtin_amdgcn_s_waitcnt(0x0F70);
             const int gy = ty0 + by;
-            float* yrow = p.y + (((size_t)n * p.H2 + min(gy, p.H2 - 1)) * p.W2 + tx0 + 4 * lhi) * p.yld + C1;
+            const size_t row_at = ((size_t)n * p.H2 + min(gy, p.H2 - 1)) * p.W2 + tx0 + 4 * lhi;
+            float* yrow = p.y + row_at * p.yld + C1;
+            _Float16* yrow_h = yh + row_at * 2 * p.yld + C1;
+            if constexpr (PLANES) {
+                const bool odd = l31 & 1;
+#pragma unroll
+                for (int nb = 0; nb < G::NB3; ++nb) {
+                    const int nn = nb * 32 + l31;
+                    float o[16];
+#pragma unroll
+                    for (int r = 0; r < 16; ++r) {
+                        const int off = (r & 3) + 8 * (r >> 2);
+                        const float v = (acc1[nb][r] + acc2[nb][r]) * inv2b;
+                        if (inner) {
+                            if (nn < C1) emax = max(emax, __float_as_uint(v) & 0x7fffffffu);
+                            o[r] = fmaxf(v, 0.f);
+                        } else {
+                            emax = max(emax, __float_as_uint(v) & 0x7fffffffu);
+                            o[r] = tx0 + 4 * lhi + off < W2n ? fmaxf(v, 0.f) : 0.f;
+                        }
+                    }
+#pragma unroll
+                    for (int r = 0; r < 16; r += 2) {
+                        const float got = __shfl_xor(odd ? o[r] : o[r + 1], 1);
+                        const int rr = odd ? r + 1 : r;
+                        const int off = (rr & 3) + 8 * (rr >> 2);
+                        const float c0 = odd ? got : o[r], c1v = odd ? o[r + 1] : got;
+                        const bool ok = nn < C1 && (inner || (gy < p.H2 && tx0 + 4 * lhi + off < p.W2));
+                        if (ok) {
+                            smax = max(smax, max(__float_as_uint(c0), __float_as_uint(c1v)) & 0x7fffffffu);
+                            f16x4 hi, lo;
+                            sf_split4(f32x4{c0, c1v, 0.f, 0.f}, neg1, hi, lo);
+                            _Float16* at = yrow_h + (size_t)off * 2 * p.yld + (nn & ~1);
+                            *reinterpret_cast<sf_f16x2*>(at) = sf_f16x2{hi[0], hi[1]};
+                            *reinterpret_cast<sf_f16x2*>(at + 2 * C1) = sf_f16x2{lo[0], lo[1]};
+                        }
+                    }
+                }
+            } else
 #pragma unroll
             for (int nb = 0; nb < G::NB3; ++nb) {
                 const int nn = nb * 32 + l31;
@@ -375,7 +437,7 @@
         }
         __syncthreads();
     }
-    if (emax >= 0x7f800000u && p.range_flag) rd_raise_flag(p.range_flag);
+    if ((emax >= 0x7f800000u || (PLANES && smax >= 0x477fe000u)) && p.range_flag) rd_raise_flag(p.range_flag);
 }
 
 bool stem_fused_supported(int c1) { return c1 == 24 || c1 == 32 || c1 == 48; }
@@ -426,16 +488,21 @@
     else sf_prepare<48>(w1, w2a, w2b, img);
 }
 
+template <int C1, bool PLANES>
+static void sf_launch_t(StemFusedParams& p, hipStream_t s, int n_cu) {
+    static unsigned long long lds_ok = 0;
+    rd_allow_dynamic_lds((const void*)stem_fused_kernel<C1, PLANES>, SfGeom<C1>::LDS_BYTES, lds_ok);
+    const int ntiles = p.N * p.tiles_x * p.tiles_y;
+    hipLaunchKernelGGL((stem_fused_kernel<C1, PLANES>), dim3(ntiles < n_cu ? ntiles : n_cu), dim3(SF_NT), SfGeom<C1>::LDS_BYTES, s, p);
+}
 template <int C1>
-static void sf_launch(StemFusedParams& p, hipStream_t s, int n_cu) {
-    static unsigned long long lds_ok = 0;
-    rd_allow_dynamic_lds((const void*)stem_fused_kernel<C1>, SfGeom<C1>::LDS_BYTES, lds_ok);
-    const int ntiles = p.N * p.tiles_x * p.tiles_y;
-    hipLaunchKernelGGL(stem_fused_kernel<C1>, dim3(ntiles < n_cu ? ntiles : n_cu), dim3(SF_NT), SfGeom<C1>::LDS_BYTES, s, p);
+static void sf_launch(StemFusedParams& p, hipStream_t s, int n_cu, bool planes) {
+    if (planes) sf_launch_t<C1, true>(p, s, n_cu);
+    else sf_launch_t<C1, false>(p, s, n_cu);
 }
 
 void launch_stem_fused(int c1, const float* x, int N, int H, int W, int in_ch, const uint16_t* wimg, const float* bias, float* y, int yld,
-                       unsigned* range_flag, hipStream_t s, const int32_t* line_tab) {
+                       unsigned* range_flag, hipStream_t s, const int32_t* line_tab, bool planes) {
     static const int n_cu = [] {
         int dev = 0, n = 256;
         (void)hipGetDevice(&dev);
@@ -453,9 +520,9 @@
     p.line_tab = line_tab;
     static const int dbg = [] { const char* e = getenv("RD_STEM_DBG"); return e ? atoi(e) : 0; }();
     p.dbg = dbg;
-    if (c1 == 24) sf_launch<24>(p, s, n_cu);
-    else if (c1 == 32) sf_launch<32>(p, s, n_cu);
-    else sf_launch<48>(p, s, n_cu);
-}
-
-}
+    if (c1 == 24) sf_launch<24>(p, s, n_cu, planes);
+    else if (c1 == 32) sf_launch<32>(p, s, n_cu, planes);
+    else sf_launch<48>(p, s, n_cu, planes);
+}
+
+}
diff --git a/rapiddoc_amd/csrc/models.cpp b/rapiddoc_amd/csrc/models.cpp
--- a/rapiddoc_amd/csrc/models.cpp
+++ b/rapiddoc_amd/csrc/models.cpp
@@ -26,7 +26,8 @@
     auto cw = [&](const char* n) { return p + "." + n + ".convolution.weight"; };
     auto bn = [&](const char* n) { return p + "." + n + ".normalization"; };
     (void)c1;
-    TView cat = b.stem_front(cw("stem1"), bn("stem1"), cw("stem2a"), bn("stem2a"), cw("stem2b"), bn("stem2b"), x_nchw);
+    const bool planes = b.stem_tail_takes_planes(cw("stem3"), bn("stem3"), cw("stem4"), bn("stem4"), x_nchw);
+    TView cat = b.stem_front(cw("stem1"), bn("stem1"), cw("stem2a"), bn("stem2a"), cw("stem2b"), bn("stem2b"), x_nchw, planes);
     TView s4 = b.stem_tail(cw("stem3"), bn("stem3"), cw("stem4"), bn("stem4"), cat, ACT_RELU, ACT_RELU);
     b.release(cat);
     (void)c2;
@@ -274,8 +275,10 @@
     const int B = x.n;
     auto cw = [&](const std::string& p) { return pre + p + ".conv.weight"; };
     auto bn = [&](const std::string& p) { return pre + p + ".bn"; };
+    const bool planes = b.stem_tail_takes_planes(cw("stem.stem3"), bn("stem.stem3"), cw("stem.stem4"), bn("stem.stem4"), x,
+                                                 cfg[0].cin + cfg[0].layers * cfg[0].mid, 0);
     TView cat = b.stem_front(cw("stem.stem1"), bn("stem.stem1"), cw("stem.stem2a"), bn("stem.stem2a"), cw("stem.stem2b"),
-                             bn("stem.stem2b"), x);
+                             bn("stem.stem2b"), x, planes);
 
     TView cur, cur_cat;
     auto new_cat = [&](int n, int h, int w, const HgStageCfg& c, int cin) { return b.alloc(n, h, w, cin + c.layers * c.mid); };
diff --git a/rapiddoc_amd/csrc/rd_kernels.h b/rapiddoc_amd/csrc/rd_kernels.h
--- a/rapiddoc_amd/csrc/rd_kernels.h
+++ b/rapiddoc_amd/csrc/rd_kernels.h
@@ -69,6 +69,7 @@
     const uint16_t* w4; float w4_inv; const float* b4;
     int act3, act4;
     unsigned* range_flag = nullptr;
+    bool x_planes = false;
     int abl = 0;
 };
 bool stem34_shape_ok(int cin, int n1, int n2);
@@ -104,7 +105,7 @@
 bool stem_fused_supported(int c1);
 void prepare_stem_fused_weights(int c1, const float* w1_stem_layout, const float* w2a_folded, const float* w2b_folded, std::vector<uint16_t>& img);
 void launch_stem_fused(int c1, const float* x, int N, int H, int W, int in_ch, const uint16_t* wimg, const float* bias, float* y, int yld,
-                       unsigned* range_flag, hipStream_t s, const int32_t* line_tab = nullptr);
+                       unsigned* range_flag, hipStream_t s, const int32_t* line_tab = nullptr, bool planes = false);
 
 constexpr int kLineTabStride = 4;
 
```

Result: no change. 346.0 (median of 5 runs) (-0.9%).
